# rockcarry/ffcnn

Measured on AMD Instinct MI355X. Metric: frames/sec yolo-fastest-1.1 @320x320 batch-64 per GPU (u8 BGR frames -> net_input's conversion in the first kernel -> full forward: conv stack + YOLO decode + NMS, boxes on rank 0), higher is better.
Workload: dtype f32

## Files before the change

### ffcnn_amd/capi.py

```python
import ctypes as C
import os
import subprocess

import numpy as np

HERE = os.path.dirname(os.path.abspath(__file__))
ROOT = os.path.dirname(HERE)
DATA = os.path.join(ROOT, "data")
CFG = os.path.join(DATA, "yolo-fastest-1.1.cfg")
WEIGHTS = os.path.join(DATA, "yolo-fastest-1.1.weights")

f32p = C.POINTER(C.c_float)


class FFGPU:
    MAX_DET = 128
    MERGE_LDS_SLOTS = 1024
    KEEP_ALL, COMPAT_V6, NO_GRAPH, NO_FUSE, HOST_DETS, SPLIT2, CONCURRENT, BF16_PW = 1, 2, 4, 8, 16, 32, 64, 128
    FEAT_FLAT, FEAT_MEAN, FEAT_MAX = 0, 1, 2
    POST_NONE, POST_SOFTMAX, POST_L2 = 0, 1, 2
    TOPK_MAX = 16
    RELABEL_KEEP_SCORE, RELABEL_LABEL_SCORE = 0, 1
    RELABEL_ENTRIES, RELABEL_MERGED = 0, 1
    K_AUTO, K_GENERIC, K_DW_STREAM, K_DW_LDS, K_PW_MFMA, K_PW_GEMM, _K6, K_DENSE_SMALL, K_IGEMM, K_PW_BF16, K_GROUP_THIN, K_PW_X3, K_CONV_X3, K_PW_X3T = range(14)
# ... 196 lines not shown
PREVIEW_KEEP_BARS = 1
PREVIEW_MAX_SIDE, PREVIEW_MAX_PANES = 8192, 4096
MOTION_DETS, MOTION_ROW, MOTION_WORDS, MOTION_MAX_SIDE = 128, 16, 8, 8192
MOTION_GATE_INVERT = 1
MOTION_ENTRIES, MOTION_MERGED = 0, 1
MOTION_ROW_HEADER = ("frame", "changed", "active", "x0", "y0", "x1", "y1", "warm")
MOTION_WORDS_HEADER = ("considered", "dropped", "outside", "moving", "warm", "frames")
MOTION_STATE_HEADER = 16
HEAT_MAX, HEAT_DETS, HEAT_ROW = 2 ** 31 - 1, 128, 8
HEAT_ANCHOR, HEAT_BOX = 0, 1
HEAT_NEAREST, HEAT_SMOOTH = 0, 1
HEAT_RAMP_ALPHA = 1
HEAT_ENTRIES, HEAT_MERGED = 0, 1
HEAT_ROW_HEADER = ("considered", "dropped", "outside", "frame", "peak", "saturated")
HEAT_STATE_HEADER = 16
TRAIL_POINTS, TRAILS_DETS, TRAILS_ROW = 32, 128, 16
TRAILS_COAST, TRAILS_TAPER = 1, 2
TRAILS_ENTRIES, TRAILS_MERGED = 0, 1
TRAILS_ROW_HEADER = ("considered", "known", "fresh", "refused", "duplicate", "anonymous", "dropped", "freed", "live", "frame", "appended", "drawn", "clipped")
TRAILS_STATE_HEADER = 16
SEG_ITEMS, SEG_LIMIT, OUTLINE_FIXED = 512, 1 << 20, 80
OUTLINE_ZONES, OUTLINE_LINES, OUTLINE_TICKS, OUTLINE_MARKERS, OUTLINE_ALARM = 1, 2, 4, 8, 16
TEXT_MAX, TEXT_ITEMS, TEXT_OPAQUE = 44, 256, 1
CAPTION_DETS = 128
CAPTION_NAME, CAPTION_SCORE, CAPTION_ID, CAPTION_OPAQUE = 1, 2, 4, 8
CAPTION_ENTRIES, CAPTION_MERGED = 0, 1
SCENE_ZONES, SCENE_LINES, ZONE_VERTS, ZONES_DETS, ZONES_ROW = 8, 8, 8, 128, 64
ZONES_NONE, ZONES_TYPE, ZONES_IDS = 0, 1, 2
ZONES_GATE_INVERT = 1
ZONES_ENTRIES, ZONES_MERGED = 0, 1
ZONES_EVENTS_HEADER = ("considered", "known", "fresh", "refused", "duplicate", "anonymous", "dropped", "freed", "live", "frame")
ZONES_STATE_HEADER = 144
TRACK_DETS = 128
TRACK_ENTRIES, TRACK_MERGED = 0, 1
TRACK_IDS_HEADER = ("considered", "matched", "born", "refused", "dropped", "freed", "live", "frame")
CROP_F32, CROP_U8 = 0, 1
CROP_ENTRIES, CROP_MERGED = 0, 1
REDACT_FILL, REDACT_MOSAIC = 0, 1
REDACT_OUTSIDE = 1
REDACT_ENTRIES, REDACT_MERGED = 0, 1
BLUR_OUTSIDE = 1
BLUR_ENTRIES, BLUR_MERGED = 0, 1
DRAW_ENTRIES, DRAW_MERGED = 0, 1
YUV_BT601_LIMITED, YUV_BT601_FULL, YUV_BT709_LIMITED, YUV_BT709_FULL = 0, 1, 2, 3

assert C.sizeof(LAYER) == 120 and C.sizeof(NET) == 104 and C.sizeof(BBOX) == 24
assert C.sizeof(FrameDets) == 16 + 24 * FFGPU.MAX_DET
assert C.sizeof(BgrFrame) == 24 and C.sizeof(Nv12Frame) == 40 and C.sizeof(Tile) == 16 and C.sizeof(TileRect) == 16
assert C.sizeof(DrawStyle) == 24 and C.sizeof(CropSpec) == 72 and C.sizeof(Crop) == 48
assert C.sizeof(TrackSpec) == 32 and C.sizeof(Track) == 48
assert C.sizeof(FeatureSpec) == 16 and C.sizeof(Label) == 8 and C.sizeof(RelabelSpec) == 16
assert C.sizeof(Gallery) == 40 and C.sizeof(RedactSpec) == 40 and C.sizeof(BlurSpec) == 40
assert C.sizeof(TextItem) == 64 and C.sizeof(CaptionSpec) == 48
assert C.sizeof(SegItem) == 32 and C.sizeof(OutlineSpec) == 40
assert C.sizeof(TrailPoint) == 12 and C.sizeof(TrailSlot) == 416 and C.sizeof(TrailsSpec) == 64
assert C.sizeof(HeatSpec) == 56 and C.sizeof(HeatBlendSpec) == 48
assert C.sizeof(MotionSpec) == 64
assert C.sizeof(Zone) == 96 and C.sizeof(Line) == 32 and C.sizeof(Scene) == 1040 and C.sizeof(ZonesSpec) == 32 and C.sizeof(ZoneSlot) == 64

BOX_DTYPE = np.dtype([("type", "<i4"), ("score", "<f4"), ("x1", "<f4"), ("y1", "<f4"), ("x2", "<f4"), ("y2", "<f4")])
DETS_DTYPE = np.dtype([("count", "<i4"), ("ncand", "<i4"), ("overflow", "<i4"), ("nfull", "<i4"),
                       ("box", BOX_DTYPE, (FFGPU.MAX_DET,))])
CROP_DTYPE = np.dtype([("target", "<i4"), ("box", "<i4"), ("type", "<i4"), ("score", "<f4"), ("x0", "<i4"), ("y0", "<i4"), ("w", "<i4"), ("h", "<i4"),
                       ("sw", "<i4"), ("sh", "<i4"), ("s1", "<i4"), ("s2", "<i4")])
TRACK_DTYPE = np.dtype([("id", "<i4"), ("type", "<i4"), ("score", "<f4"), ("x1", "<f4"), ("y1", "<f4"), ("x2", "<f4"), ("y2", "<f4"),
                        ("hits", "<i4"), ("missed", "<i4"), ("born", "<i4"), ("det", "<i4"), ("reserved", "<i4")])
ZONE_SLOT_DTYPE = np.dtype([("id", "<i4"), ("px", "<f4"), ("py", "<f4"), ("inside", "<i4"), ("last", "<i4"), ("reserved", "<i4", (3,)), ("since", "<i4", (8,))])
TRAIL_POINT_DTYPE = np.dtype([("x", "<i4"), ("y", "<i4"), ("frame", "<i4")])
TRAIL_SLOT_DTYPE = np.dtype([("id", "<i4"), ("last", "<i4"), ("n", "<i4"), ("head", "<i4"), ("cx", "<i4"), ("cy", "<i4"), ("reserved", "<i4", (2,)),
                             ("ring", TRAIL_POINT_DTYPE, (32,))])
LABEL_DTYPE = np.dtype([("index", "<i4"), ("value", "<f4")])
TEXT_ITEM_DTYPE = np.dtype([("x", "<i4"), ("y", "<i4"), ("fg", "u1", (4,)), ("bg", "u1", (4,)), ("scale", "u1"), ("flags", "u1"), ("len", "u1"), ("reserved", "u1"),
                            ("text", "u1", (44,))])
SEG_ITEM_DTYPE = np.dtype([("x0", "<i4"), ("y0", "<i4"), ("x1", "<i4"), ("y1", "<i4"), ("color", "u1", (4,)), ("thickness", "u1"), ("dash", "u1"), ("flags", "u1"),
                           ("reserved", "u1"), ("reserved2", "<i4", (2,))])

EXPORTS = ["net_load", "net_free", "net_input", "net_forward", "net_dump", "net_profile", "groupconv",
           "ffgpu_device_count", "ffgpu_set_device", "ffgpu_last_error", "ffgpu_build_info",
           "ffgpu_net_weights_dev", "ffgpu_net_weights_commit",
           "ffgpu_exec_create", "ffgpu_exec_destroy", "ffgpu_exec_batch", "ffgpu_exec_arena_bytes",
           "ffgpu_exec_kernel_count", "ffgpu_exec_work_model", "ffgpu_exec_set_scale", "ffgpu_exec_forward_dev", "ffgpu_exec_forward_host",
           "ffgpu_exec_forward_bgr_dev", "ffgpu_exec_forward_bgr_frames_dev", "ffgpu_exec_forward_nv12_frames_dev", "ffgpu_exec_dets_dev", "ffgpu_exec_dets_host", "ffgpu_exec_set_ring", "ffgpu_exec_set_ring_strided", "ffgpu_exec_read_dets", "ffgpu_exec_read_layer", "ffgpu_exec_hash_layers",
           "ffgpu_exec_read_boxes", "ffgpu_exec_cand_capacity", "ffgpu_exec_graph_captures",
           "ffgpu_exec_profile", "ffgpu_exec_profile_steps", "ffgpu_exec_step_model", "ffgpu_groupconv_dev", "ffgpu_groupconv_kernel_name", "ffgpu_groupconv_time_dev", "ffgpu_irb_dev", "ffgpu_irb_flags_dev", "ffgpu_irb_plan_text", "ffgpu_irb_thin_launch_text", "ffgpu_irb_stage_plan_text", "ffgpu_front_plan_text", "ffgpu_irb_instantiations", "ffgpu_knobs_text", "ffgpu_dwpw_dev", "ffgpu_packed_records_bytes", "ffgpu_pack_records", "ffgpu_unpack_records",
           "ffgpu_shard_range", "ffgpu_node_create", "ffgpu_node_destroy", "ffgpu_node_ndev", "ffgpu_node_shard", "ffgpu_node_set_scale",
           "ffgpu_node_input_dev", "ffgpu_node_input_slot_dev", "ffgpu_node_depth", "ffgpu_node_rccl_ranks", "ffgpu_node_forward", "ffgpu_node_forward_host",
           "ffgpu_node_submit", "ffgpu_node_wait", "ffgpu_node_run",
           "ffgpu_merge_tiles_scratch_bytes", "ffgpu_merge_tiles_dev", "ffgpu_exec_merge_tiles", "ffgpu_exec_merged_dev", "ffgpu_exec_read_merged",
           "ffgpu_exec_read_merged_boxes", "ffgpu_tile_plan",
           "ffgpu_draw_boxes_bgr_dev", "ffgpu_draw_boxes_nv12_dev", "ffgpu_exec_draw_bgr", "ffgpu_exec_draw_nv12",
           "ffgpu_crop_table_bytes", "ffgpu_crop_slot_bytes", "ffgpu_crop_boxes_bgr_dev", "ffgpu_crop_boxes_nv12_dev", "ffgpu_exec_crop_bgr", "ffgpu_exec_crop_nv12",
           "ffgpu_crops_to_source_dev",
           "ffgpu_track_state_bytes", "ffgpu_track_reset_dev", "ffgpu_track_boxes_dev", "ffgpu_exec_track",
           "ffgpu_feature_dim", "ffgpu_exec_feature_dim", "ffgpu_features_dev", "ffgpu_exec_features", "ffgpu_topk_dev", "ffgpu_crops_relabel_dev",
           "ffgpu_exec_relabel",
           "ffgpu_match_workspace_bytes", "ffgpu_match_dev", "ffgpu_gallery_enroll_dev",
           "ffgpu_redact_boxes_bgr_dev", "ffgpu_redact_boxes_nv12_dev", "ffgpu_exec_redact_bgr", "ffgpu_exec_redact_nv12",
           "ffgpu_blur_boxes_bgr_dev", "ffgpu_blur_boxes_nv12_dev", "ffgpu_exec_blur_bgr", "ffgpu_exec_blur_nv12",
           "ffgpu_zones_state_bytes", "ffgpu_scene_check", "ffgpu_zones_reset_dev", "ffgpu_zones_boxes_dev", "ffgpu_exec_zones",
           "ffgpu_font_builtin", "ffgpu_draw_text_bgr_dev", "ffgpu_draw_text_nv12_dev", "ffgpu_caption_boxes_dev", "ffgpu_exec_caption_bgr", "ffgpu_exec_caption_nv12",
           "ffgpu_caption_scene_dev",
           "ffgpu_draw_segments_bgr_dev", "ffgpu_draw_segments_nv12_dev", "ffgpu_outline_spec_check", "ffgpu_outline_scene_dev",
           "ffgpu_trails_state_bytes", "ffgpu_trails_spec_check", "ffgpu_trails_reset_dev", "ffgpu_trails_boxes_dev", "ffgpu_exec_trails",
           "ffgpu_heat_state_bytes", "ffgpu_heat_spec_check", "ffgpu_heat_blend_spec_check", "ffgpu_heat_palette", "ffgpu_heat_reset_dev", "ffgpu_heat_boxes_dev",
           "ffgpu_exec_heat", "ffgpu_heat_blend_bgr_dev", "ffgpu_heat_blend_nv12_dev",
           "ffgpu_motion_state_bytes", "ffgpu_motion_spec_check", "ffgpu_motion_reset_dev", "ffgpu_motion_update_bgr_dev", "ffgpu_motion_update_nv12_dev",
           "ffgpu_motion_gate_dev", "ffgpu_exec_motion_gate",
           "ffgpu_preview_spec_check", "ffgpu_preview_rect", "ffgpu_preview_grid", "ffgpu_preview_tile", "ffgpu_preview_bgr_dev", "ffgpu_preview_nv12_dev",
           "ffgpu_warp_spec_check", "ffgpu_warp_mesh_size", "ffgpu_warp_mesh_orient", "ffgpu_warp_mesh_homography", "ffgpu_warp_mesh_lens", "ffgpu_warp_point",
           "ffgpu_warp_tile", "ffgpu_warp_bgr_dev", "ffgpu_warp_nv12_dev"]
DIAG_EXPORTS = ["ffgpu_membench", "ffgpu_pipe_probe", "ffgpu_pipe_probe2", "ffgpu_pipe_probe3", "ffgpu_mfma_floor", "ffgpu_diag_x3_term", "ffgpu_diag_xl_op", "ffgpu_clock_probe"]


def library_path():
    return os.environ.get("FFCNN_HIP_LIB") or os.path.join(HERE, "lib", "libffcnn_hip.so")


def build_library(force=False):
    cmd = ["make", "-C", os.path.join(HERE, "csrc")]
    if force:
        subprocess.check_call(cmd + ["clean"], stdout=subprocess.DEVNULL)
    subprocess.check_call(cmd, stdout=subprocess.DEVNULL)
    return library_path()


_lib = None


def lib():
    global _lib
    if _lib is not None:
        return _lib
    path = library_path()
    if not os.path.exists(path):
        raise RuntimeError("%s is missing: run `python -c 'import __graft_entry__ as g; g.build()'` "
                           "(the HIP extension is the only compute path)" % path)
    L = C.CDLL(path)
    vp, i, sz = C.c_void_p, C.c_int, C.c_size_t
    L.net_load.restype = C.POINTER(NET)
    L.net_load.argtypes = [C.c_char_p, C.c_char_p, i, i]
    L.net_free.argtypes = [C.POINTER(NET)]
    L.net_input.argtypes = [C.POINTER(NET), vp, i, i, f32p, f32p]
    L.net_forward.argtypes = [C.POINTER(NET)]
    L.net_dump.argtypes = [C.POINTER(NET)]
    L.net_profile.argtypes = [C.POINTER(NET)]
    L.groupconv.argtypes = [f32p, f32p, f32p] + [i] * 12 + [C.POINTER(f32p), C.POINTER(i)]
    L.ffgpu_last_error.restype = C.c_char_p
    L.ffgpu_build_info.restype = C.c_char_p
    if b" DIAG " in L.ffgpu_build_info() and os.environ.get("FFCNN_HIP_ALLOW_DIAG") != "1":
        raise RuntimeError("%s is a DIAG (lab) build of libffcnn_hip; set FFCNN_HIP_ALLOW_DIAG=1 to load it on purpose" % path)
    L.ffgpu_set_device.argtypes = [i]
    L.ffgpu_net_weights_dev.argtypes = [C.POINTER(NET), C.POINTER(vp), C.POINTER(sz)]
    L.ffgpu_net_weights_commit.argtypes = [C.POINTER(NET), vp]
    L.ffgpu_exec_create.restype = vp
    L.ffgpu_exec_create.argtypes = [C.POINTER(NET), i, i]
    L.ffgpu_exec_destroy.argtypes = [vp]
    L.ffgpu_exec_batch.argtypes = [vp]
    L.ffgpu_exec_arena_bytes.restype = sz
    L.ffgpu_exec_arena_bytes.argtypes = [vp]
    L.ffgpu_exec_kernel_count.argtypes = [vp]
    L.ffgpu_exec_work_model.argtypes = [vp, C.POINTER(C.c_double), C.POINTER(C.c_double)]
    L.ffgpu_exec_set_scale.argtypes = [vp, i, i]
    L.ffgpu_exec_forward_dev.argtypes = [vp, vp, vp]
    L.ffgpu_exec_forward_host.argtypes = [vp, f32p]
    L.ffgpu_exec_forward_bgr_dev.argtypes = [vp, vp, i, i, f32p, f32p, vp]
    L.ffgpu_exec_forward_bgr_frames_dev.argtypes = [vp, C.POINTER(BgrFrame), i, f32p, f32p, vp]
    L.ffgpu_exec_forward_nv12_frames_dev.argtypes = [vp, C.POINTER(Nv12Frame), i, f32p, f32p, vp]
    L.ffgpu_exec_dets_dev.argtypes = [vp, C.POINTER(vp), C.POINTER(sz)]
    L.ffgpu_exec_dets_host.restype = vp; L.ffgpu_exec_dets_host.argtypes = [vp]
    L.ffgpu_exec_set_ring.argtypes = [vp, vp, C.c_int]
    L.ffgpu_exec_set_ring_strided.argtypes = [vp, vp, C.c_int, C.c_int]
    L.ffgpu_exec_read_dets.argtypes = [vp, vp, i]
    L.ffgpu_exec_read_layer.argtypes = [vp, i, i, f32p, sz]
    L.ffgpu_exec_hash_layers.argtypes = [vp, vp, i]
    L.ffgpu_exec_profile.argtypes = [vp, vp, f32p]
    L.ffgpu_exec_profile_steps.argtypes = [vp, vp, C.POINTER(i), f32p, i]
    L.ffgpu_exec_step_model.argtypes = [vp, C.POINTER(i), C.POINTER(C.c_double), i]
    L.ffgpu_groupconv_dev.argtypes = [vp, vp, vp] + [i] * 15 + [vp]
    L.ffgpu_groupconv_kernel_name.restype = C.c_char_p
    L.ffgpu_groupconv_kernel_name.argtypes = [i] * 10
    L.ffgpu_groupconv_time_dev.restype = C.c_float
    L.ffgpu_groupconv_time_dev.argtypes = [vp, vp, vp] + [i] * 17 + [vp]
    L.ffgpu_irb_dev.restype = C.c_float
    L.ffgpu_irb_dev.argtypes = [vp] * 6 + [i] * 13 + [vp]
    L.ffgpu_irb_flags_dev.restype = C.c_float
    L.ffgpu_irb_flags_dev.argtypes = [vp] * 6 + [i] * 14 + [vp]
    L.ffgpu_irb_thin_launch_text.argtypes = [i] * 12 + [C.c_char_p, i]
    L.ffgpu_irb_plan_text.argtypes = [i] * 12 + [C.c_char_p, i]
    L.ffgpu_irb_stage_plan_text.argtypes = [i] * 7 + [C.c_char_p, i]
    L.ffgpu_front_plan_text.argtypes = [i] * 4 + [C.c_char_p, i]
    L.ffgpu_irb_instantiations.argtypes = [C.c_char_p, i]
    L.ffgpu_knobs_text.argtypes = [C.c_char_p, i]
    L.ffgpu_exec_read_boxes.argtypes = [vp, i, vp, i]
    L.ffgpu_exec_cand_capacity.argtypes = [vp]
    L.ffgpu_exec_graph_captures.argtypes = [vp]
    L.ffgpu_dwpw_dev.restype = C.c_float
    L.ffgpu_dwpw_dev.argtypes = [vp] * 4 + [i] * 10 + [vp]
    L.ffgpu_packed_records_bytes.restype = C.c_size_t
    L.ffgpu_packed_records_bytes.argtypes = [i, i]
    L.ffgpu_pack_records.restype = i
    L.ffgpu_pack_records.argtypes = [vp, i, C.c_long, i, i, vp, vp]
    L.ffgpu_shard_range.argtypes = [i, i, i, C.POINTER(i), C.POINTER(i)]
    L.ffgpu_shard_range.restype = None
    L.ffgpu_node_create.restype = vp
    L.ffgpu_node_create.argtypes = [C.POINTER(NET), i, C.POINTER(i), i, i, i]
    L.ffgpu_node_destroy.argtypes = [vp]
    L.ffgpu_node_ndev.argtypes = [vp]
    L.ffgpu_node_shard.argtypes = [vp, i, C.POINTER(i), C.POINTER(i), C.POINTER(i)]
    L.ffgpu_node_set_scale.argtypes = [vp, i, i]
    L.ffgpu_node_input_dev.restype = vp
    L.ffgpu_node_input_dev.argtypes = [vp, i]
    L.ffgpu_node_input_slot_dev.restype = vp
    L.ffgpu_node_input_slot_dev.argtypes = [vp, i, i]
    L.ffgpu_node_depth.argtypes = [vp]
    if hasattr(L, "ffgpu_node_rccl_ranks"):
        L.ffgpu_node_rccl_ranks.argtypes = [vp]
    L.ffgpu_node_submit.restype = C.c_long
    L.ffgpu_node_submit.argtypes = [vp, f32p]
    L.ffgpu_node_wait.argtypes = [vp, C.c_long, vp]
    L.ffgpu_node_run.argtypes = [vp, C.c_long, vp]
    L.ffgpu_unpack_records.argtypes = [vp, i, i, vp]
    L.ffgpu_node_forward.argtypes = [vp, vp]
    L.ffgpu_node_forward_host.argtypes = [vp, f32p, vp]
    L.ffgpu_merge_tiles_scratch_bytes.restype = sz
    L.ffgpu_merge_tiles_scratch_bytes.argtypes = [i, i]
    L.ffgpu_merge_tiles_dev.argtypes = [vp, vp, i, C.POINTER(Tile), i, i, C.c_float, i, vp, vp, vp, sz, vp]
    L.ffgpu_exec_merge_tiles.argtypes = [vp, C.POINTER(Tile), i, i, vp]
    L.ffgpu_exec_merged_dev.argtypes = [vp, C.POINTER(vp), C.POINTER(sz)]
    L.ffgpu_exec_read_merged.argtypes = [vp, vp, i]
    L.ffgpu_exec_read_merged_boxes.argtypes = [vp, i, vp, i]
    L.ffgpu_tile_plan.argtypes = [i] * 7 + [C.POINTER(TileRect), i]
    L.ffgpu_draw_boxes_bgr_dev.argtypes = [vp, vp, i, C.POINTER(i), C.POINTER(BgrFrame), i, C.POINTER(DrawStyle), vp]
    L.ffgpu_draw_boxes_nv12_dev.argtypes = [vp, vp, i, C.POINTER(i), C.POINTER(Nv12Frame), i, C.POINTER(DrawStyle), vp]
    L.ffgpu_exec_draw_bgr.argtypes = [vp, i, C.POINTER(BgrFrame), i, C.POINTER(DrawStyle), vp]
    L.ffgpu_exec_draw_nv12.argtypes = [vp, i, C.POINTER(Nv12Frame), i, C.POINTER(DrawStyle), vp]
    L.ffgpu_redact_boxes_bgr_dev.argtypes = [vp, vp, i, C.POINTER(i), C.POINTER(BgrFrame), i, C.POINTER(RedactSpec), vp]
    L.ffgpu_redact_boxes_nv12_dev.argtypes = [vp, vp, i, C.POINTER(i), C.POINTER(Nv12Frame), i, C.POINTER(RedactSpec), vp]
    L.ffgpu_exec_redact_bgr.argtypes = [vp, i, C.POINTER(BgrFrame), i, C.POINTER(RedactSpec), vp]
    L.ffgpu_exec_redact_nv12.argtypes = [vp, i, C.POINTER(Nv12Frame), i, C.POINTER(RedactSpec), vp]
    L.ffgpu_blur_boxes_bgr_dev.argtypes = [vp, vp, i, C.POINTER(i), C.POINTER(BgrFrame), C.POINTER(BgrFrame), i, C.POINTER(BlurSpec), vp]
    L.ffgpu_blur_boxes_nv12_dev.argtypes = [vp, vp, i, C.POINTER(i), C.POINTER(Nv12Frame), C.POINTER(Nv12Frame), i, C.POINTER(BlurSpec), vp]
    L.ffgpu_exec_blur_bgr.argtypes = [vp, i, C.POINTER(BgrFrame), C.POINTER(BgrFrame), i, C.POINTER(BlurSpec), vp]
    L.ffgpu_exec_blur_nv12.argtypes = [vp, i, C.POINTER(Nv12Frame), C.POINTER(Nv12Frame), i, C.POINTER(BlurSpec), vp]
    L.ffgpu_crop_table_bytes.restype = sz
    L.ffgpu_crop_table_bytes.argtypes = [i]
    L.ffgpu_crop_slot_bytes.restype = sz
    L.ffgpu_crop_slot_bytes.argtypes = [i, i, i]
    L.ffgpu_crop_boxes_bgr_dev.argtypes = [vp, vp, i, C.POINTER(i), C.POINTER(BgrFrame), i, C.POINTER(CropSpec), vp, vp, i, vp]
    L.ffgpu_crop_boxes_nv12_dev.argtypes = [vp, vp, i, C.POINTER(i), C.POINTER(Nv12Frame), i, C.POINTER(CropSpec), vp, vp, i, vp]
    L.ffgpu_exec_crop_bgr.argtypes = [vp, i, C.POINTER(BgrFrame), i, C.POINTER(CropSpec), vp, vp, i, vp]
    L.ffgpu_exec_crop_nv12.argtypes = [vp, i, C.POINTER(Nv12Frame), i, C.POINTER(CropSpec), vp, vp, i, vp]
    L.ffgpu_crops_to_source_dev.argtypes = [vp, i, vp, vp, i, vp, vp, vp]
    L.ffgpu_track_state_bytes.restype = sz
    L.ffgpu_track_state_bytes.argtypes = [i, i]
    L.ffgpu_track_reset_dev.argtypes = [vp, i, i, i, vp]
    L.ffgpu_track_boxes_dev.argtypes = [vp, vp, i, C.POINTER(i), C.POINTER(i), i, C.POINTER(TrackSpec), vp, i, vp, vp, vp, vp]
    L.ffgpu_exec_track.argtypes = [vp, i, C.POINTER(i), i, C.POINTER(TrackSpec), vp, i, vp, vp, vp, vp]
    L.ffgpu_zones_state_bytes.restype = sz
    L.ffgpu_zones_state_bytes.argtypes = [i, i]
    L.ffgpu_scene_check.argtypes = [C.POINTER(Scene), i]
    L.ffgpu_zones_reset_dev.argtypes = [vp, i, i, i, vp]
    L.ffgpu_zones_boxes_dev.argtypes = [vp, vp, i, C.POINTER(i), C.POINTER(i), i, C.POINTER(ZonesSpec), vp, vp, i, vp, vp, vp, vp, vp]
    L.ffgpu_exec_zones.argtypes = [vp, i, C.POINTER(i), i, C.POINTER(ZonesSpec), vp, vp, i, vp, vp, vp, vp, vp]
    L.ffgpu_font_builtin.restype = None
    L.ffgpu_font_builtin.argtypes = [vp]
    L.ffgpu_draw_text_bgr_dev.argtypes = [vp, i, vp, C.POINTER(BgrFrame), i, vp]
    L.ffgpu_draw_text_nv12_dev.argtypes = [vp, i, vp, C.POINTER(Nv12Frame), i, vp]
    L.ffgpu_caption_boxes_dev.argtypes = [vp, vp, i, C.POINTER(i), i, C.POINTER(CaptionSpec), vp, vp, i, vp]
    L.ffgpu_exec_caption_bgr.argtypes = [vp, i, C.POINTER(BgrFrame), i, C.POINTER(CaptionSpec), vp, vp, i, vp, vp]
    L.ffgpu_exec_caption_nv12.argtypes = [vp, i, C.POINTER(Nv12Frame), i, C.POINTER(CaptionSpec), vp, vp, i, vp, vp]
# ... 1172 lines not shown
                                     act, flags, variant, stream), "ffgpu_groupconv_dev")


def groupconv_time_dev(d_in, d_filt, d_out, batch, iw, ih, ic, groups, pad, stride, fs, fn, act=0, flags=0, variant=0,
                       warmup=5, iters=20, stream=None):
    ow, oh = (iw + 2 * pad - fs) // stride + 1, (ih + 2 * pad - fs) // stride + 1
    us = lib().ffgpu_groupconv_time_dev(d_in, d_filt, d_out, batch, iw, ih, ic, groups, pad, stride, fs, fn, ow, oh, fn,
                                        act, flags, variant, warmup, iters, stream)
    if us < 0:
        raise RuntimeError("ffgpu_groupconv_time_dev failed: %s" % last_error())
    return us


def packed_records_bytes(batch, cap):
    return int(lib().ffgpu_packed_records_bytes(batch, cap))


def pack_records_dev(d_records, nslots, slot_stride_records, batch, cap, d_out, stream=None):
    _check(lib().ffgpu_pack_records(d_records, nslots, slot_stride_records, batch, cap, d_out, stream), "ffgpu_pack_records")


def kernel_name(batch, iw, ih, ic, groups, pad, stride, fs, fn, variant=0):
    return lib().ffgpu_groupconv_kernel_name(batch, iw, ih, ic, groups, pad, stride, fs, fn, variant).decode()


def irb_plan_text(shape, flags=0):
    buf = C.create_string_buffer(1024)
    if lib().ffgpu_irb_plan_text(*shape, flags, buf, len(buf)) < 0:
        raise RuntimeError("ffgpu_irb_plan_text failed: %s" % last_error())
    return buf.value.decode()


def irb_stage_plan_text(batch, iw, ih, blocks, act1=2, actd=2, flags=0):
    buf = C.create_string_buffer(1024)
    if lib().ffgpu_irb_stage_plan_text(batch, iw, ih, blocks, act1, actd, flags, buf, len(buf)) < 0:
        raise RuntimeError("ffgpu_irb_stage_plan_text failed: %s" % last_error())
    return buf.value.decode()


FRONT_FORMS = {"f32": 0, "u8": 1, "bgr_frames": 2, "nv12_frames": 3}


def front_plan_text(batch, pw, ph, form="f32"):
    buf = C.create_string_buffer(256)
    if lib().ffgpu_front_plan_text(batch, pw, ph, FRONT_FORMS[form], buf, len(buf)) < 0:
        raise RuntimeError("ffgpu_front_plan_text failed: %s" % last_error())
    return buf.value.decode()


def irb_instantiations():
    buf = C.create_string_buffer(4096)
    n = lib().ffgpu_irb_instantiations(buf, len(buf))
    if n < 0 or n >= len(buf):
        raise RuntimeError("ffgpu_irb_instantiations failed: %s" % (last_error() if n < 0 else "%d bytes" % n))
    return buf.value.decode().split()


def knobs():
    buf = C.create_string_buffer(1 << 16)
    n = lib().ffgpu_knobs_text(buf, len(buf))
    if n < 0 or n >= len(buf):
        raise RuntimeError("ffgpu_knobs_text failed: %s" % (last_error() if n < 0 else "%d bytes" % n))
    rows = []
    for line in buf.value.decode().splitlines():
        name, kind, dflt, cls, value, text = line.split(" ", 5)
        rows.append({"name": name, "kind": kind, "default": None if dflt == "-" else dflt if dflt == "computed" else int(dflt), "cls": cls, "value": value, "text": text})
    return rows


def dwpw_dev(d_in, d_wd, d_wp, d_out, batch, iw, ih, c, oc, fs, actd=2, actp=0, warmup=0, iters=0, stream=None):
    us = lib().ffgpu_dwpw_dev(d_in, d_wd, d_wp, d_out, batch, iw, ih, c, oc, fs, actd, actp, warmup, iters, stream)
    if us < 0:
        raise RuntimeError("ffgpu_dwpw_dev failed: %s" % last_error())
    return us


def irb_thin_launch_text(shape, flags=0):
    buf = C.create_string_buffer(256)
    if lib().ffgpu_irb_thin_launch_text(*shape, flags, buf, len(buf)) < 0:
        raise RuntimeError("ffgpu_irb_thin_launch_text failed: %s" % last_error())
    return buf.value.decode()


def irb_dev(d_in, d_w1, d_wd, d_w2, d_res, d_out, batch, iw, ih, ic, ec, oc, stride, act1=2, actd=2, act2=0, res_act=0,
            warmup=0, iters=0, stream=None, flags=0):
    us = lib().ffgpu_irb_flags_dev(d_in, d_w1, d_wd, d_w2, d_res, d_out, batch, iw, ih, ic, ec, oc, stride, act1, actd, act2, res_act, flags,
                                   warmup, iters, stream)
    if us < 0:
        raise RuntimeError("ffgpu_irb_dev failed: %s" % last_error())
    return us


def preview_pane(src=None, dst=None):
    p = PreviewPane()
    if src is not None:
        p.sx, p.sy, p.sw, p.sh = (int(v) for v in src)
    if dst is not None:
        p.dx, p.dy, p.dw, p.dh = (int(v) for v in dst)
    return p


def preview_spec(fit=PREVIEW_STRETCH, fill=(0, 0, 0), keep_bars=False):
    sp = PreviewSpec()
    sp.fit, sp.flags = fit, PREVIEW_KEEP_BARS if keep_bars else 0
    sp.fill[:] = (int(fill[0]), int(fill[1]), int(fill[2]), 0)
    return sp


def preview_spec_check(spec):
    _check(lib().ffgpu_preview_spec_check(spec), "ffgpu_preview_spec_check")


def preview_rect(src_w, src_h, dst_w, dst_h, pane, spec, nv12=False):
    out = (C.c_int * 8)()
    _check(lib().ffgpu_preview_rect(src_w, src_h, dst_w, dst_h, pane, spec, int(bool(nv12)), out), "ffgpu_preview_rect")
    return tuple(out)


def preview_grid(npanes, cols, dst_w, dst_h, gap=0, nv12=False):
    arr = (PreviewPane * max(1, npanes))()
    _check(lib().ffgpu_preview_grid(npanes, cols, dst_w, dst_h, gap, int(bool(nv12)), arr), "ffgpu_preview_grid")
    return [PreviewPane.from_buffer_copy(arr[k]) for k in range(npanes)]


def preview_tile():
    out = (C.c_int * 3)()
    _check(lib().ffgpu_preview_tile(out), "ffgpu_preview_tile")
    return tuple(out)


def _preview_panes(panes):
    arr = (PreviewPane * max(1, len(panes)))()
    for k, p in enumerate(panes):
        arr[k] = p
    return arr


def preview_bgr_dev(srcs, dsts, panes, spec, stream=None):
    if not len(srcs) == len(dsts) == len(panes):
        raise ValueError("%d sources, %d destinations and %d panes" % (len(srcs), len(dsts), len(panes)))
    _check(lib().ffgpu_preview_bgr_dev(bgr_frame_table(srcs), bgr_frame_table(dsts), _preview_panes(panes), len(panes), spec, stream), "ffgpu_preview_bgr_dev")


def preview_nv12_dev(srcs, dsts, panes, spec, stream=None):
    if not len(srcs) == len(dsts) == len(panes):
        raise ValueError("%d sources, %d destinations and %d panes" % (len(srcs), len(dsts), len(panes)))
    _check(lib().ffgpu_preview_nv12_dev(nv12_frame_table(srcs), nv12_frame_table(dsts), _preview_panes(panes), len(panes), spec, stream), "ffgpu_preview_nv12_dev")


def warp_spec(filter=WARP_BILINEAR, border=WARP_FILL, fill=(0, 0, 0)):
    sp = WarpSpec()
    sp.filter, sp.border = filter, border
    sp.fill[:] = (int(fill[0]), int(fill[1]), int(fill[2]), 0)
    return sp


def warp_spec_check(spec):
    _check(lib().ffgpu_warp_spec_check(spec), "ffgpu_warp_spec_check")


def warp_mesh_size(dst_w, dst_h, cell):
    out = (C.c_int * 2)()
    _check(lib().ffgpu_warp_mesh_size(dst_w, dst_h, cell, out), "ffgpu_warp_mesh_size")
    return tuple(out)


# ... 71 lines not shown
```

### ffcnn_amd/csrc/ffgpu_conv_kernels.inc

```
#include "ffgpu_dw_stream.inc"
#include "ffgpu_pw_mfma.inc"
#include "ffgpu_pw_gemm32.inc"
#include "ffgpu_pw_bf16.inc"
#include "ffgpu_conv_igemm.inc"
#include "ffgpu_dwpw.inc"
#include "ffgpu_conv_dense.inc"
#include "ffgpu_irb.inc"
#include "ffgpu_irb_thin.inc"
#include "ffgpu_front.inc"
#include "ffgpu_irb_wave.inc"
#include "ffgpu_irb_wave2.inc"
#include "ffgpu_irb_stage.inc"
#include "ffgpu_pw_x3.inc"
#include "ffgpu_pw_x3t.inc"
#include "ffgpu_conv_x3.inc"
#include "ffgpu_dw_lds.inc"
#include "ffgpu_dw_pair.inc"
#include "ffgpu_conv_thin.inc"

struct BareScratch {
    float *p = nullptr; size_t n = 0; int dev = -1;
    float *get(size_t need)
    {
        int d = 0;
// ... 975 lines not shown
}

static ThinP thin_params(const IrbDesc &d)
{
    ThinP p;
    p.in = d.in; p.out = d.out; p.residual = d.residual; p.w1 = d.w1; p.wd = d.wd; p.w2 = d.w2;
    p.W = d.W; p.H = d.H; p.N = d.N;
    p.band = d.plan.band; p.nbands = (d.H + p.band - 1) / p.band;
    p.act1 = act_slope(d.act1); p.actd = act_slope(d.actd); p.act2 = act_slope(d.act2); p.res_act = act_slope(d.res_act);
    p.ntasks = (long)d.N * p.nbands;
    return p;
}

template <int IC, int EC, int OC>
static int irb_thin_launch(const ThinP &p, const IrbPlan &c, hipStream_t s)
{
    hipLaunchKernelGGL((k_irb_thin<IC, EC, OC>), dim3((unsigned)c.grid), dim3(c.block), 0, s, p);
    LAUNCH_OK("irb_thin");
    return 0;
}

static constexpr bool thin_pair_built(int ic, int ncp) { return !(ic == 8 && ncp == 5); }
static int thin_pair_ncp(int W, int ic)
{
    for (int nc = 3; nc <= 5; nc++)
        if (W % nc == 0 && W / nc <= 32) return thin_pair_built(ic, nc) ? nc : 0;
    return 0;
}

struct ThinForm { int ncp, band, nbands; long ntasks; int grid; };
static ThinForm thin_form(const IrbDesc &d)
{
    ThinForm f;
    const int ncp = thin_pair_ncp(d.W, d.ic);
    const bool pair = ncp && d.N >= 2 && (d.flags & FFGPU_CONCURRENT) && knob(K_THIN_PAIR) != 0;
    const int units = pair ? (d.N + 1) / 2 : d.N;
    f.ncp = pair ? ncp : 0;
    f.band = pair ? knob_or(K_THIN_BAND, thin_band(units, d.H)) : d.plan.band;
    f.nbands = (d.H + f.band - 1) / f.band;
    f.ntasks = (long)units * f.nbands;
    f.grid = pair ? (int)((f.ntasks + 3) / 4) : d.plan.grid;
    return f;
}

template <int IC, int EC, int OC>
static int irb_thin_pair_launch(const ThinP &p, const ThinForm &f, hipStream_t s)
{
    if (f.ncp == 3) hipLaunchKernelGGL((k_irb_thin_pair<IC, EC, OC, 3>), dim3((unsigned)f.grid), dim3(256), 0, s, p);
    else if (f.ncp == 4) hipLaunchKernelGGL((k_irb_thin_pair<IC, EC, OC, 4>), dim3((unsigned)f.grid), dim3(256), 0, s, p);
    else if constexpr (thin_pair_built(IC, 5)) hipLaunchKernelGGL((k_irb_thin_pair<IC, EC, OC, 5>), dim3((unsigned)f.grid), dim3(256), 0, s, p);
    else { ffgpu_set_error("irb_thin_pair: no instantiation for %d columns per lane of %d channels", f.ncp, IC); return -1; }
    LAUNCH_OK("irb_thin_pair");
    return 0;
}

typedef int (*IrbThinLaunch)(const ThinP &, const IrbPlan &, hipStream_t);
typedef int (*IrbThinPairLaunch)(const ThinP &, const ThinForm &, hipStream_t);
struct IrbThinKernel { int IC, OC; IrbThinLaunch launch; IrbThinPairLaunch pair; };
static const IrbThinKernel irb_thin_kernels[] = { { 8, 4, irb_thin_launch<8, 8, 4>, irb_thin_pair_launch<8, 8, 4> }, { 4, 4, irb_thin_launch<4, 8, 4>, irb_thin_pair_launch<4, 8, 4> },
                                                  { 8, 8, irb_thin_launch<8, 8, 8>, irb_thin_pair_launch<8, 8, 8> }, { 4, 8, irb_thin_launch<4, 8, 8>, irb_thin_pair_launch<4, 8, 8> } };

static int launch_irb_thin(const IrbDesc &d, hipStream_t s)
{
    ThinP p = thin_params(d);
    const ThinForm f = thin_form(d);
    if (f.ncp) { p.band = f.band; p.nbands = f.nbands; p.ntasks = f.ntasks; }
    for (const IrbThinKernel &k : irb_thin_kernels)
        if (k.IC == d.ic && k.OC == d.oc) return f.ncp ? k.pair(p, f, s) : k.launch(p, d.plan, s);
    ffgpu_set_error("irb_thin: no instantiation for %d -> 8 -> %d channels", d.ic, d.oc);
    return -1;
}

int ffgpu_irb_thin_launch_line(const IrbDesc &d, char *buf, size_t cap)
{
    if (d.plan.family != IRB_THIN) return snprintf(buf, cap, "unsupported");
    const ThinForm f = thin_form(d);
    char key[48];
    if (f.ncp) snprintf(key, sizeof key, "thin_pair<%d,8,%d,%d>", d.ic, d.oc, f.ncp);
    else snprintf(key, sizeof key, "thin<%d,8,%d>", d.ic, d.oc);
    return snprintf(buf, cap, "%s W=%d H=%d N=%d band=%d nbands=%d ntasks=%ld grid=%d block=256", key, d.W, d.H, d.N, f.band, f.nbands, f.ntasks, f.grid);
}

typedef int (*IrbwLaunch)(const IrbwP &, const IrbPlan &, hipStream_t);
struct IrbwKernel { int KS1, OT, S, NSI, NSO; bool big, x3, xl; Knob gate; IrbwLaunch launch; };
#define IRBW_K(ks1, ot, st, nsi, gate) \
    { ks1, ot, st, nsi, 1, true, false, false, gate, irb_launch_t<IrbwP, k_irbw<ks1, ot, st, nsi, true>> }, \
    { ks1, ot, st, nsi, 1, false, false, false, gate, irb_launch_t<IrbwP, k_irbw<ks1, ot, st, nsi, false>> }
static const IrbwKernel irbw_kernels[] = {
    { 2, 1, 1, 3, 2, true, true, false, K_NONE, irb_launch_t<IrbwP, k_irbw2<2, 3, true>> }, { 4, 1, 1, 3, 2, true, true, false, K_NONE, irb_launch_t<IrbwP, k_irbw2<4, 3, true>> },
    { 2, 1, 1, 3, 2, true, false, false, K_NONE, irb_launch_t<IrbwP, k_irbw2<2, 3, false>> }, { 4, 1, 1, 3, 2, true, false, false, K_NONE, irb_launch_t<IrbwP, k_irbw2<4, 3, false>> },
    { 12, 3, 1, 2, 1, true, true, true, K_NONE, irb_launch_t<IrbwP, k_irbw<12, 3, 1, 2, true, true, true>> },
    { 4, 2, 2, 4, 1, true, true, false, K_NONE, irb_launch_t<IrbwP, k_irbw<4, 2, 2, 4, true, true>> },
    { 6, 2, 1, 2, 1, true, true, false, K_NONE, irb_launch_t<IrbwP, k_irbw<6, 2, 1, 2, true, true>> },
    IRBW_K(1, 1, 1, 2, K_NONE), IRBW_K(2, 1, 1, 2, K_NONE), IRBW_K(4, 1, 1, 2, K_NONE), IRBW_K(2, 2, 1, 2, K_NONE), IRBW_K(4, 2, 1, 2, K_NONE),
    IRBW_K(6, 2, 1, 2, K_NONE), IRBW_K(12, 3, 1, 2, K_NONE), IRBW_K(1, 1, 2, 3, K_NONE), IRBW_K(2, 1, 2, 3, K_NONE), IRBW_K(4, 2, 2, 4, K_NONE),
    IRBW_K(6, 3, 2, 3, K_IRBW_S2_633),
    IRBW_K(1, 1, 2, 4, K_IRBW_S2_NSI4), IRBW_K(2, 1, 2, 4, K_IRBW_S2_NSI4),
};
#undef IRBW_K
static const int irbw_nkernels = (int)(sizeof irbw_kernels / sizeof irbw_kernels[0]);

static bool irbw_has_kernel(int KS1, int OT, int S, int NSI)
{
    for (const IrbwKernel &k : irbw_kernels)
        if (k.KS1 == KS1 && k.OT == OT && k.S == S && k.NSI == NSI && k.NSO == 1 && !k.x3) return k.gate == K_NONE || knob(k.gate) != 0;
    return false;
}

static long irbw_ntiles(const IrbDesc &d, int TWq, int TH) { return (long)d.N * ((d.OW + 4 * TWq - 1) / (4 * TWq)) * ((d.OH + TH - 1) / TH); }

static bool irbw_pick(const IrbDesc &d, IrbPlan &c)
{
    if (knob(K_NO_IRBW)) return false;
    if (d.stride != 1 && d.stride != 2) return false;
    if (d.act1 == 3 || d.actd == 3 || d.act2 == 3 || d.res_act == 3) return false;
    if ((size_t)d.ic * d.N * d.H * d.W >= (1u << 30) || (size_t)d.oc * d.N * d.OH * d.OW >= (1u << 30)) return false;
    const int S = d.stride;
    c.KS1 = ((d.ic + 3) & ~3) / 4; c.OT = (d.oc + 15) / 16; c.ngroups = (d.ec + 15) / 16;
    double best = 1e30;
    for (int TWq = 1; TWq <= 8; TWq++) {
        if (TWq > 1 && (TWq - 1) * 4 >= d.OW) break;
        for (int TH = 1; TWq * TH <= 16 && TH <= d.OH + 1; TH++) {
            const int EW = S == 1 ? 4 * TWq + 4 : 8 * TWq + 4, EH = S * (TH - 1) + 3;
            int NSI = (EW * EH + 63) / 64;
            if (NSI < 2) NSI = 2;
            if (S == 2 && NSI < 3) NSI = 3;
            if (NSI > 4 || !irbw_has_kernel(c.KS1, c.OT, S, NSI)) continue;
            const long tiles = irbw_ntiles(d, TWq, TH) / d.N;
            const double cost = (double)tiles * (NSI * (c.KS1 * 128.0 + 500.0) + 4 * (220.0 + c.OT * 128.0)) * (1.0 + 12.0 / EW);
            if (cost < best) { best = cost; c.TWq = TWq; c.TH = TH; c.EW = EW; c.EH = EH; c.NSI = NSI; }
        }
    }
    if (best > 1e29) return false;
    const int ft = knob(K_IRBW_TWQ), fh = knob(K_IRBW_TH);
    if (ft > 0 && fh > 0 && ft * fh <= 16) {
        const int EW = S == 1 ? 4 * ft + 4 : 8 * ft + 4, EH = S * (fh - 1) + 3;
        if (EW * EH <= c.NSI * 64) { c.TWq = ft; c.TH = fh; c.EW = EW; c.EH = EH; }
    }
    const long ntiles = irbw_ntiles(d, c.TWq, c.TH);
    const int regs = c.NSI * c.KS1 * 4 + c.OT * 16 + 2 * (c.KS1 + 4 * c.OT) + 76;
    c.big = regs > 124;
    if (const int f = knob(K_IRBW_BIG); f >= 0) c.big = f != 0;
    if (const int f = S == 2 && c.KS1 == 1 ? knob(K_IRBW_BIG_S2K1) : -1; f >= 0) c.big = f != 0;
    const bool conc = (d.flags & FFGPU_CONCURRENT) != 0;
    const int x3_mask = knob(K_IRBW_X3);
    const int gmax = std::min(8, c.ngroups);
    int G = 1;
    for (int g = 1; g <= gmax; g++) {
        const size_t slot = (size_t)c.OT * 1024, ereg = (size_t)g * 16 * c.NSI * 64;
        if (g > 1 && ereg / slot < (size_t)(g + 1) / 2) continue;
        G = g;
        if (ntiles * g >= knob_or(K_IRBW_GWAVES, conc ? 500 : 1200)) break;
    }
    if (!conc && G > 1 && G < gmax && c.ngroups % G != 0 && (c.ngroups + G) / (G + 1) <= (c.ngroups + G - 1) / G) G++;
    if (d.stride == 1 && c.ngroups == 9 && ntiles >= 400 && ntiles < 512 && gmax >= 4 && !conc && !knob(K_IRBW_NOEXC)) G = 4;
    if (const int f = ntiles >= 256 && ntiles < 1100 ? knob(K_IRBW_G_MID) : 0; f > 0) G = std::min(gmax, f);
    const bool xl_ok = S == 1 && c.KS1 == 12 && c.OT == 3 && c.NSI == 2 && c.big && ((x3_mask >> 3) & 1) != 0;
    if (xl_ok && conc && ntiles < 256) G = std::min(gmax, knob(K_IRBW_G_XL));
    if (const int f = ntiles < 256 ? knob(K_IRBW_G_SMALL) : 0; f > 0) G = std::min(gmax, f);
    const int fg = knob(K_IRBW_G);
    if (fg >= 1 && fg <= gmax) G = fg;
    c.G = G;
    c.NSO = 1;
    c.x3 = S == 1 && c.KS1 == 6 && c.OT == 2 && c.NSI == 2 && c.big && ((x3_mask >> 2) & 1) != 0;
    if (S == 2 && c.KS1 == 4 && c.OT == 2 && c.NSI == 4 && c.big && ((x3_mask >> 4) & 1) != 0) c.x3 = true;
    c.xl = xl_ok && G > 1;
    if (c.xl) c.x3 = true;
    if (G == 1 && S == 1 && c.OT == 1 && (c.KS1 == 2 || c.KS1 == 4) && knob(K_IRBW_NSO) == 2) {
        double best2 = 1e30; int tw2 = 0, th2 = 0;
        for (int TWq = 1; TWq <= 8; TWq++) {
            if (TWq > 1 && (TWq - 1) * 4 >= d.OW) break;
            for (int TH = 1; TWq * TH <= 32 && TH <= d.OH + 1; TH++) {
                if (TWq * TH <= 16 || TWq * ((TH + 1) / 2) > 16) continue;
                const int EW = 4 * TWq + 4, EH = TH + 2;
                if (EW * EH > 192) continue;
                const long tiles = irbw_ntiles(d, TWq, TH) / d.N;
                const double cost = (double)tiles * (3 * (c.KS1 * 128.0 + 500.0) + 2 * 4 * (220.0 + 128.0)) * (1.0 + 12.0 / EW);
                if (cost < best2) { best2 = cost; tw2 = TWq; th2 = TH; }
            }
        }
        const int f2t = knob(K_IRBW2_TWQ), f2h = knob(K_IRBW2_TH);
        if (f2t > 0 && f2h > 0 && f2t * ((f2h + 1) / 2) <= 16 && (4 * f2t + 4) * (f2h + 2) <= 192) { tw2 = f2t; th2 = f2h; best2 = 0; }
        const long nt2 = tw2 ? irbw_ntiles(d, tw2, th2) : 0;
// ... 331 lines not shown
}

size_t ffgpu_irb_pack_floats(const IrbDesc &d) { return irb_planned(d, "irb_pack_floats") ? (size_t)d.plan.pack_floats : 0; }

int ffgpu_irb_pack(const IrbDesc &d, float *pk, hipStream_t s)
{
    const IrbPlan &c = d.plan;
    if (!irb_planned(d, "irb_pack")) return -1;
    if (c.family == IRB_THIN) return 0;
    if (c.family == IRB_WAVE) {
        IrbwPackP q; q.w1 = d.w1; q.wd = d.wd; q.w2 = d.w2; q.pk = pk; q.ic = d.ic; q.ec = d.ec; q.oc = d.oc;
        q.k4 = (d.ic + 3) & ~3; q.OT = c.OT; q.ngroups = c.ngroups; q.x3 = c.x3; q.half = c.half;
        hipLaunchKernelGGL(k_irbw_pack, dim3((c.pack_floats + 255) / 256), dim3(256), 0, s, q);
        LAUNCH_OK("irbw_pack");
        return 0;
    }
    IrbPackP q;
    q.w1 = d.w1; q.wd = d.wd; q.w2 = d.w2; q.pk = pk;
    q.ic = d.ic; q.ec = d.ec; q.oc = d.oc;
    q.k4 = (d.ic + 3) & ~3; q.ECH = c.ECH; q.MT = c.ECH / 16; q.OT = c.OT; q.nchunks = (d.ec + c.ECH - 1) / c.ECH; q.CH = irb_chunk_floats(q.k4, c.ECH, c.OT);
    const int total = q.nchunks * q.CH + q.OT * 32;
    hipLaunchKernelGGL(k_irb_pack, dim3((total + 255) / 256), dim3(256), 0, s, q);
    LAUNCH_OK("irb_pack");
    return 0;
}

static int irb_thin_key(int ic, int oc, char *key, size_t cap) { return snprintf(key, cap, "thin<%d,8,%d>", ic, oc); }
static int irbw_key(const IrbwKernel &k, char *key, size_t cap)
{
    if (k.NSO == 2) return snprintf(key, cap, "irbw2<%d,%d%s>", k.KS1, k.NSI, k.x3 ? ",x3" : "");
    return snprintf(key, cap, "irbw<%d,%d,%d,%d%s%s%s>", k.KS1, k.OT, k.S, k.NSI, k.big ? ",big" : "", k.x3 ? ",x3" : "", k.xl ? ",xl" : "");
}
static int irb_key(const IrbKernel &k, char *key, size_t cap) { return snprintf(key, cap, "irb<%d,%d,%d,%d,%d>", k.MT, k.OT, k.S, k.NW == 8 ? 1 : 2, k.NW); }

int ffgpu_irb_keys(char *buf, size_t cap)
{
    size_t n = 0;
    char key[48];
    auto put = [&]() { n += (size_t)snprintf(n < cap ? buf + n : nullptr, n < cap ? cap - n : 0, "%s\n", key); };
    for (const IrbThinKernel &k : irb_thin_kernels) { irb_thin_key(k.IC, k.OC, key, sizeof key); put(); }
    for (const IrbwKernel &k : irbw_kernels) { irbw_key(k, key, sizeof key); put(); }
    for (const IrbKernel &k : irb_kernels) { irb_key(k, key, sizeof key); put(); }
    return (int)n;
}

int ffgpu_irb_plan_line(const IrbDesc &d, char *buf, size_t cap)
{
    const IrbPlan &c = d.plan;
    char key[48];
    if (c.family == IRB_THIN) {
        const ThinP p = thin_params(d);
        irb_thin_key(d.ic, d.oc, key, sizeof key);
        return snprintf(buf, cap, "%s W=%d H=%d N=%d band=%d nbands=%d act=%g,%g,%g,%g ntasks=%ld lds=%d grid=%d block=%d half=%d pack=%d",
                        key, p.W, p.H, p.N, p.band, p.nbands, p.act1, p.actd, p.act2, p.res_act, p.ntasks, c.lds, c.grid, c.block, c.half, c.pack_floats);
    }
    if (c.family == IRB_WAVE) {
        const IrbwP p = irbw_params(d);
        const IrbwKernel &k = irbw_kernels[c.inst];
        irbw_key(k, key, sizeof key);
        return snprintf(buf, cap, "%s N=%d H=%d W=%d OH=%d OW=%d ic=%d ec=%d oc=%d act=%g,%g,%g,%g tile=%d,%d,%d,%d tiles=%d,%d,%ld ngroups=%d G=%d WPB=%d o_w2=%d o_cs=%d cs_floats=%d "
                        "xl_off=%d red_cap=%d in_elems=%u vec=%d half_last=%d m=%u,%u,%u,%u xcd=%d lds=%d grid=%d block=%d half=%d pack=%d",
                        key, p.N, p.H, p.W, p.OH, p.OW, p.ic, p.ec, p.oc, p.act1, p.actd, p.act2, p.res_act, p.TWq, p.TH, p.EW, p.EH, p.tiles_x, p.tiles_y, p.ntiles, p.ngroups, p.G, p.WPB,
                        p.o_w2, p.o_cs, p.cs_floats, p.xl_off, p.red_cap, p.in_elems, p.vec, p.half_last, p.m_ew, p.m_tx, p.m_ty, p.m_twq, p.xcd, c.lds, c.grid, c.block, c.half, c.pack_floats);
    }
    if (c.family == IRB_WG) {
        const IrbP p = irb_params(d);
        const IrbKernel &k = irb_kernels[c.inst];
        irb_key(k, key, sizeof key);
        return snprintf(buf, cap, "%s N=%d H=%d W=%d OH=%d OW=%d ic=%d ec=%d oc=%d stride=%d act=%g,%g,%g,%g tile=%d,%d,%d,%d,%d,%d NPin=%d NPout=%d tiles=%d,%d,%d "
                        "k4=%d nchunks=%d ECH=%d CH=%d KS=%d red_off=%d vec_store=%d resident=%d inv_nsi=%d lds=%d grid=%d block=%d half=%d pack=%d",
                        key, p.N, p.H, p.W, p.OH, p.OW, p.ic, p.ec, p.oc, p.stride, p.act1, p.actd, p.act2, p.res_act, p.TH, p.TW, p.TWq, p.NF, p.EH, p.EW,
                        p.NPin, p.NPout, p.tiles_x, p.tiles_y, p.ntiles, p.k4, p.nchunks, p.ECH, p.CH, p.KS, p.red_off, p.vec_store, p.resident, p.inv_nsi, c.lds, c.grid, c.block, c.half, c.pack_floats);
    }
    return snprintf(buf, cap, "unsupported");
}

int ffgpu_launch_irb(const IrbDesc &d, hipStream_t s)
{
    const IrbPlan &c = d.plan;
    if (!irb_planned(d, "irb")) return -1;
    if (knob(K_VERBOSE_IRB)) { char line[1024]; ffgpu_irb_plan_line(d, line, sizeof line); fprintf(stderr, "%s\n", line); }
    if (c.family == IRB_THIN) return launch_irb_thin(d, s);
    if (!d.pk) { ffgpu_set_error("irb: constants not packed"); return -1; }
    return c.family == IRB_WAVE ? irbw_kernels[c.inst].launch(irbw_params(d), c, s) : irb_kernels[c.inst].launch(irb_params(d), c, s);
}

static bool irb_stage_params(const IrbDesc *blocks, int B, IrbStageP &p, size_t &lds)
{
    if (B < 2 || B > IRBS_MAXB) return false;
    const IrbDesc &d0 = blocks[0];
    for (int b = 0; b < B; b++) {
        const IrbDesc &d = blocks[b];
        const IrbPlan &c = d.plan;
        if (d.ic != 48 || d.ec != 224 || d.oc != 48 || d.stride != 1 || d.OH != d.H || d.OW != d.W) return false;
        if (d.N != d0.N || d.H != d0.H || d.W != d0.W || d.act1 != d0.act1 || d.actd != d0.actd) return false;
        if (act_slope(d.act2) != 1.f || act_slope(d.res_act) != 1.f) return false;
        if (c.family != IRB_WAVE || !c.xl || !c.x3 || c.half || c.G != IRBS_WAVES || c.KS1 != 12 || c.OT != 3 || c.ngroups != 2 * IRBS_WAVES) return false;
        if (c.region / (c.OT * 1024) < c.G) return false;
    }
    const int plane = d0.H * d0.W, TWq = (d0.W + 3) / 4;
    if (plane > 128 || TWq * d0.H > 32) return false;
    p = IrbStageP{};
    p.B = B; p.N = d0.N; p.H = d0.H; p.W = d0.W;
    p.act1 = act_slope(d0.act1); p.actd = act_slope(d0.actd);
    p.TWq = TWq; p.P = 4 * TWq + 2; p.EP = p.P * (d0.H + 2);
    int total;
    irbw_layout(d0.plan, p.o_w2, p.o_cs, p.cs_floats, total);
    if (p.cs_floats > 2 * IRBS_WAVES * 64 * 4) return false;
    p.e_off = p.cs_floats;
    p.e_slice = std::max(16 * p.EP, 2048);
    p.xi_off = p.e_off + IRBS_WAVES * p.e_slice;
    p.f_off = p.xi_off + 2 * 4 * 64 * IRBW_XL_DW;
    lds = (size_t)(p.f_off + 48 * plane) * sizeof(float);
    p.m_w = umulhi_magic(d0.W); p.m_twq = umulhi_magic(TWq); p.m_plane = umulhi_magic(plane);
    return lds <= IRB_LDS_MAX;
}

bool ffgpu_irb_stage_ok(const IrbDesc *blocks, int B)
{
    IrbStageP p; size_t lds;
    return irb_stage_params(blocks, B, p, lds);
}

int ffgpu_irb_stage_line(const IrbDesc *blocks, int B, bool wanted, char *buf, size_t cap)
{
    IrbStageP p; size_t lds;
    if (!wanted || !irb_stage_params(blocks, B, p, lds)) return snprintf(buf, cap, "blocks B=%d launches=%d", B, B);
    return snprintf(buf, cap, "stage B=%d launches=1 N=%d H=%d W=%d act=%g,%g TWq=%d P=%d EP=%d o_w2=%d o_cs=%d cs_floats=%d e_off=%d e_slice=%d xi_off=%d f_off=%d m=%u,%u,%u lds=%zu grid=%d block=%d",
                    p.B, p.N, p.H, p.W, p.act1, p.actd, p.TWq, p.P, p.EP, p.o_w2, p.o_cs, p.cs_floats, p.e_off, p.e_slice, p.xi_off, p.f_off, p.m_w, p.m_twq, p.m_plane, lds, p.N, IRBS_WAVES * 64);
}

int ffgpu_launch_irb_stage(const IrbDesc *blocks, int B, hipStream_t s)
{
    IrbStageP p; size_t lds;
    if (!irb_stage_params(blocks, B, p, lds)) { ffgpu_set_error("irb_stage: the run of %d blocks does not fit the stage kernel", B); return -1; }
    p.in = blocks[0].in; p.out = blocks[B - 1].out;
    for (int b = 0; b < B; b++) {
        if (!blocks[b].pk) { ffgpu_set_error("irb_stage: constants not packed"); return -1; }
        p.pk[b] = blocks[b].pk;
    }
    if (!p.in || !p.out) { ffgpu_set_error("irb_stage: no tensors"); return -1; }
    if (lds_allow((const void *)k_irb_stage, lds, "irb_stage")) return -1;
    hipLaunchKernelGGL(k_irb_stage, dim3((unsigned)p.N), dim3(IRBS_WAVES * 64), lds, s, p);
    LAUNCH_OK("irb_stage");
    return 0;
}
```

### ffcnn_amd/csrc/ffgpu_dev.hpp

```cpp
#pragma once
#include <hip/hip_runtime.h>
#include <stddef.h>
#include <stdint.h>
#include <vector>
#include "ffgpu_internal.h"
#include "ffgpu_args.hpp"
#include "ffgpu_streams_host.hpp"
#include "ffgpu_track_host.hpp"
#include "ffgpu_zones_host.hpp"
#include "ffgpu_text_host.hpp"
#include "ffgpu_lines_host.hpp"
#include "ffgpu_trails_host.hpp"
#include "ffgpu_heat_host.hpp"
#include "ffgpu_motion_host.hpp"
#include "ffgpu_preview_host.hpp"
#include "ffgpu_warp_host.hpp"

#define FFGPU_CHECK(expr)                                                                   \
    do {                                                                                    \
        hipError_t e_ = (expr);                                                             \
        if (e_ != hipSuccess) {                                                             \
            ffgpu_set_error("%s failed: %s (%s:%d)", #expr, hipGetErrorString(e_), __FILE__, __LINE__); \
            return -1;                                                                      \
        }                                                                                   \
    } while (0)

struct ConvDesc {
    const float *in;
    const float *const *in_ind;
    const float *filt;
    float       *out;
    const float *residual;
    const float *wpack;
    int   N;
    int   iw, ih, ic;
    int   ow, oh, oc;
    int   fs, stride, pad, groups;
    int   act;
    int   res_act;
    int   flags;
    long  in_cs, in_ns, out_cs, out_ns, res_cs, res_ns;
    int   nsplit;
    int   kernel;
    int   x3_mt;
};
#define FFGPU_F_BATCH_INPUT (1 << 30)

static inline int conv_k4(const ConvDesc &d) { return (d.fs * d.fs * (d.ic / d.groups) + 3) & ~3; }

enum { IRB_NONE = 0, IRB_THIN, IRB_WAVE, IRB_WG };
struct IrbPlan {
    int family;
    int inst;
    int half;
    int pack_floats;
    int lds, grid, block;
    int KS1, OT, NSI, NSO, TWq, TH, EW, EH, ngroups, G, WPB, big, x3, xl;
    int xcd, region;
    int TW, NF, ECH, NW, KS, wbufs, red_off;
    int band, front_band;
};
struct IrbDesc {
    const float *in; float *out; const float *residual;
    const float *w1, *wd, *w2;
    int N, H, W, OH, OW, ic, ec, oc, stride;
    int act1, actd, act2, res_act;
    const float *pk;
    int flags;
    IrbPlan plan;
};
bool   ffgpu_irb_plan(IrbDesc &d);
size_t ffgpu_irb_pack_floats(const IrbDesc &d);
int    ffgpu_irb_pack(const IrbDesc &d, float *pk, hipStream_t s);
int    ffgpu_launch_irb(const IrbDesc &d, hipStream_t s);
int    ffgpu_irb_plan_line(const IrbDesc &d, char *buf, size_t cap);
int    ffgpu_irb_thin_launch_line(const IrbDesc &d, char *buf, size_t cap);
int    ffgpu_irb_keys(char *buf, size_t cap);
#define IRBS_MAXB 8
bool   ffgpu_irb_stage_ok(const IrbDesc *blocks, int B);
int    ffgpu_launch_irb_stage(const IrbDesc *blocks, int B, hipStream_t s);
int    ffgpu_irb_stage_line(const IrbDesc *blocks, int B, bool wanted, char *buf, size_t cap);
bool   ffgpu_front_ok(const ConvDesc &c, const IrbDesc &d);
enum InputForm { IN_F32, IN_U8, IN_BGR_FRAMES, IN_NV12_FRAMES, IN_FORMS };
int    ffgpu_launch_front(const ConvDesc &c, const IrbDesc &d, InputForm form, hipStream_t s);
bool   ffgpu_front_nv12_fused();
int    ffgpu_front_plan_line(const IrbDesc &d, InputForm form, char *buf, size_t cap);
int    ffgpu_front_nc(const IrbDesc &d);

bool   ffgpu_dwpw_ok(const ConvDesc &dw, const ConvDesc &pw);
size_t ffgpu_dwpw_pack_floats(const ConvDesc &dw, const ConvDesc &pw);
int    ffgpu_dwpw_pack(const ConvDesc &dw, const ConvDesc &pw, float *pk, hipStream_t s);
int    ffgpu_launch_dwpw(const ConvDesc &dw, const ConvDesc &pw, const float *wpack, hipStream_t s);

size_t ffgpu_pw_pack_floats(const ConvDesc &d);
void   ffgpu_conv_plan(ConvDesc &d);
int    ffgpu_pw_pack(const ConvDesc &d, float *pk, hipStream_t s);

#define FFGPU_YUV_MATRICES { { 16, 298, 409, 100, 208, 516 }, { 0, 256, 359, 88, 183, 454 }, { 16, 298, 459, 55, 136, 541 }, { 0, 256, 403, 48, 120, 475 } }
int  ffgpu_launch_set_frames(FrameDesc *d_tab, const FrameDesc *h_desc, int n, hipStream_t s);
int  ffgpu_launch_input_frames(const FrameDesc *d_tab, bool nv12, float *out, int N, int W, int H, const float mean[3], const float norm[3], hipStream_t s);

struct ExecParams {
    const float *frames;
    int s1, s2;
    ffgpu_frame_dets *ring;
    int ring_slots, ring_stride;
    int bbox_max;
    const unsigned char *bgr;
    long  bgr_frame;
    int   bgr_pitch;
    float mean[3], norm[3];
    const FrameDesc *frames_tab;
};
int  ffgpu_launch_set_params(ExecParams *d_prm, const ExecParams &v, hipStream_t s);
bool ffgpu_conv_supports_ind(const ConvDesc &d);

bool ffgpu_no_device(const char *what);

int         ffgpu_launch_conv(const ConvDesc &d, int variant, hipStream_t s);
const char *ffgpu_conv_kernel_name(const ConvDesc &d, int variant);
int ffgpu_launch_pool(const float *in, float *out, int N, int c, int w, int h, int fs, int stride, int is_max, hipStream_t s);
int ffgpu_launch_spp(const float *in, float *const out[3], const int fs[3], int n, long planes, int w, int h, hipStream_t s);
int ffgpu_launch_upsample(const float *in, float *out, long planes, int w, int h, int stride, hipStream_t s);
int ffgpu_launch_add_act(const float *a, const float *b, float *out, long n, int act, hipStream_t s);
int ffgpu_launch_copy(const float *src, float *dst, long n, hipStream_t s);
int ffgpu_launch_hash64(const float *x, long n, unsigned long long *out, hipStream_t s);
int ffgpu_launch_input_bgr(const unsigned char *bgr, float *out, int N, int w, int h, int W, int H,
                           int sw, int sh, int s1, int s2, const float mean[3], const float norm[3], hipStream_t s);

struct YoloHead {
    const float *in;
    int   w, h, classes;
    int   anchors[3][2];
    float thresh, scale_xy;
    int   key_base;
};
int ffgpu_launch_yolo(const YoloHead &hd, int N, int netw, int neth, BBOX *cand, int *cand_key, int *ncand, int cap, int *ring_ctr, hipStream_t s);
int ffgpu_launch_nms(const BBOX *cand, const int *cand_key, int *ncand, int cap, BBOX *full, void *scratch,
                     ffgpu_frame_dets *dets, ffgpu_frame_dets *dets_host, const int *ring_ctr, int N,
                     float thresh, int use_min, const ExecParams *prm, hipStream_t s);
#define FFGPU_NMS_LDS_CAP 8192
bool ffgpu_nms_in_lds(int cap_pow2);
int ffgpu_launch_clear(int *ncand, int N, int *ring_ctr, hipStream_t s);

int    ffgpu_merge_build_tab(const char *what, const ffgpu_tile *tiles, int ntiles, int nimages, std::vector<int> &tab, std::vector<int> *off);
size_t ffgpu_merge_tab_bytes(int ntiles);
int    ffgpu_launch_set_ints(int *d_dst, const int *h_src, int n, hipStream_t s);
int    ffgpu_launch_merge_tiles(const int *d_tab, const std::vector<int> &tab, const ffgpu_frame_dets *recs, const BBOX *lists, int stride,
                                float thresh, int use_min, ffgpu_frame_dets *out_recs, BBOX *out_lists, void *scratch, hipStream_t s);

int ffgpu_draw_style_check(const char *what, const ffgpu_draw_style *st, unsigned pal[256], int *npal);
int ffgpu_launch_draw(bool nv12, const DetSource &src, const std::vector<DrawTarget> &targets, const unsigned pal[256], int npal, int thickness, hipStream_t s);

struct CropPlan {
    int   out_w, out_h, form, per_target, nclasses, num, den;
    float min_score, mean[3], norm[3];
    unsigned char classes[256];
};
// ... 50 lines not shown
```

### ffcnn_amd/csrc/ffgpu_exec.hip

```cpp
#include <algorithm>
#include <cstdarg>
#include <cstdint>
#include <cstdio>
#include <cstdlib>
#include <cstring>
#include <map>
#include <mutex>
#include <string>
#include <type_traits>
#include <vector>

#include "ffgpu_dev.hpp"
#include "ffgpu_knobs.hpp"
#include "ffgpu_plan.hpp"
#include "conv.h"

static thread_local char g_err[512] = "";

extern "C" void ffgpu_set_error(const char *fmt, ...)
{
    va_list ap;
    va_start(ap, fmt);
    vsnprintf(g_err, sizeof g_err, fmt, ap);
    va_end(ap);
// ... 1744 lines not shown
{
    if (iters < 1 || fn != oc) { ffgpu_set_error("groupconv_time_dev: bad arguments"); return -1.f; }
    hipStream_t s = (hipStream_t)stream;
    ConvDesc d;
    fill_desc(d, d_in, d_filt, d_out, batch, iw, ih, ic, groups, pad, stride, fs, ow, oh, oc, act, flags);
    float *pk = nullptr;
    if (variant == FFGPU_K_AUTO && ffgpu_pw_pack_floats(d) > 0) {
        if (hipMalloc(&pk, ffgpu_pw_pack_floats(d) * sizeof(float)) != hipSuccess || ffgpu_pw_pack(d, pk, s)) { ffgpu_set_error("pack failed"); return -1.f; }
        d.wpack = pk;
    }
    hipEvent_t e0, e1;
    if (hipEventCreate(&e0) != hipSuccess || hipEventCreate(&e1) != hipSuccess) { ffgpu_set_error("hipEventCreate failed"); return -1.f; }
    for (int i = 0; i < warmup; i++) if (ffgpu_launch_conv(d, variant, s)) return -1.f;
    (void)hipEventRecord(e0, s);
    for (int i = 0; i < iters; i++) if (ffgpu_launch_conv(d, variant, s)) return -1.f;
    (void)hipEventRecord(e1, s);
    if (hipEventSynchronize(e1) != hipSuccess) { ffgpu_set_error("hipEventSynchronize: %s", hipGetErrorString(hipGetLastError())); return -1.f; }
    float ms = 0.f;
    (void)hipEventElapsedTime(&ms, e0, e1);
    (void)hipEventDestroy(e0); (void)hipEventDestroy(e1);
    return ms * 1000.f / iters;
}

static void irb_fill(IrbDesc &d, int batch, int iw, int ih, int ic, int ec, int oc, int stride, int act1, int actd, int act2, int res_act)
{
    d.N = batch; d.H = ih; d.W = iw; d.OH = (ih + 2 - 3) / stride + 1; d.OW = (iw + 2 - 3) / stride + 1;
    d.ic = ic; d.ec = ec; d.oc = oc; d.stride = stride;
    d.act1 = act1; d.actd = actd; d.act2 = act2; d.res_act = res_act;
}

extern "C" int ffgpu_irb_plan_text(int batch, int iw, int ih, int ic, int ec, int oc, int stride, int act1, int actd, int act2, int res_act, int flags, char *buf, int cap)
{
    if (!buf || cap < 1 || batch < 1 || iw < 1 || ih < 1 || stride < 1) { ffgpu_set_error("irb_plan_text: bad arguments"); return -1; }
    IrbDesc d{};
    irb_fill(d, batch, iw, ih, ic, ec, oc, stride, act1, actd, act2, res_act);
    d.flags = flags & FFGPU_CONCURRENT;
    (void)ffgpu_irb_plan(d);
    return ffgpu_irb_plan_line(d, buf, (size_t)cap);
}

extern "C" int ffgpu_front_plan_text(int batch, int pw, int ph, int form, char *buf, int cap)
{
    if (!buf || cap < 1 || batch < 1 || pw < 1 || ph < 1 || form < 0 || form >= IN_FORMS) { ffgpu_set_error("front_plan_text: bad arguments"); return -1; }
    IrbDesc d{};
    irb_fill(d, batch, pw, ph, 8, 8, 4, 1, 0, 0, 0, 0);
    if (!ffgpu_irb_plan(d) || d.plan.family != IRB_THIN) return snprintf(buf, (size_t)cap, "unsupported");
    return ffgpu_front_plan_line(d, (InputForm)form, buf, (size_t)cap);
}

extern "C" int ffgpu_irb_stage_plan_text(int batch, int iw, int ih, int blocks, int act1, int actd, int flags, char *buf, int cap)
{
    if (!buf || cap < 1 || batch < 1 || iw < 1 || ih < 1 || blocks < 1 || blocks > 64) { ffgpu_set_error("irb_stage_plan_text: bad arguments"); return -1; }
    std::vector<IrbDesc> run((size_t)blocks, IrbDesc{});
    for (IrbDesc &d : run) {
        irb_fill(d, batch, iw, ih, 48, 224, 48, 1, act1, actd, 0, 0);
        d.flags = flags & FFGPU_CONCURRENT;
        if (!ffgpu_irb_plan(d)) return snprintf(buf, (size_t)cap, "unsupported");
    }
    return ffgpu_irb_stage_line(run.data(), blocks, stage_wanted(batch, flags), buf, (size_t)cap);
}

extern "C" int ffgpu_irb_instantiations(char *buf, int cap)
{
    if (!buf || cap < 1) { ffgpu_set_error("irb_instantiations: bad arguments"); return -1; }
    return ffgpu_irb_keys(buf, (size_t)cap);
}

extern "C" int ffgpu_knobs_text(char *buf, int cap)
{
    if (!buf || cap < 1) { ffgpu_set_error("knobs_text: bad arguments"); return -1; }
    return ffgpu_knobs_lines(buf, (size_t)cap);
}

extern "C" int ffgpu_irb_thin_launch_text(int batch, int iw, int ih, int ic, int ec, int oc, int stride, int act1, int actd, int act2, int res_act, int flags, char *buf, int cap)
{
    if (!buf || cap < 1 || batch < 1 || iw < 1 || ih < 1 || stride < 1) { ffgpu_set_error("irb_thin_launch_text: bad arguments"); return -1; }
    IrbDesc d{};
    irb_fill(d, batch, iw, ih, ic, ec, oc, stride, act1, actd, act2, res_act);
    d.flags = flags & FFGPU_CONCURRENT;
    (void)ffgpu_irb_plan(d);
    return ffgpu_irb_thin_launch_line(d, buf, (size_t)cap);
}

extern "C" float ffgpu_irb_dev(const float *d_in, const float *d_w1, const float *d_wd, const float *d_w2,
                               const float *d_res, float *d_out, int batch, int iw, int ih, int ic, int ec, int oc,
                               int stride, int act1, int actd, int act2, int res_act, int warmup, int iters, void *stream)
{
    return ffgpu_irb_flags_dev(d_in, d_w1, d_wd, d_w2, d_res, d_out, batch, iw, ih, ic, ec, oc, stride, act1, actd, act2, res_act, 0, warmup, iters, stream);
}

extern "C" float ffgpu_irb_flags_dev(const float *d_in, const float *d_w1, const float *d_wd, const float *d_w2,
                                     const float *d_res, float *d_out, int batch, int iw, int ih, int ic, int ec, int oc,
                                     int stride, int act1, int actd, int act2, int res_act, int flags, int warmup, int iters, void *stream)
{
    hipStream_t s = (hipStream_t)stream;
    IrbDesc d{};
    d.in = d_in; d.out = d_out; d.residual = d_res; d.w1 = d_w1; d.wd = d_wd; d.w2 = d_w2;
    irb_fill(d, batch, iw, ih, ic, ec, oc, stride, act1, actd, act2, res_act);
    d.flags = flags & FFGPU_CONCURRENT;
    if (!d_in || !d_out || !d_w1 || !d_wd || !d_w2 || !ffgpu_irb_plan(d)) { ffgpu_set_error("irb_dev: unsupported block shape"); return -1.f; }
    float *pk = nullptr;
    if (hipMalloc(&pk, ffgpu_irb_pack_floats(d) * sizeof(float)) != hipSuccess) { ffgpu_set_error("irb_dev: hipMalloc failed"); return -1.f; }
    d.pk = pk;
    float us = 0.f;
    int rc = ffgpu_irb_pack(d, pk, s);
    if (!rc && iters <= 0) rc = ffgpu_launch_irb(d, s);
    if (!rc && iters > 0) {
        hipEvent_t e0, e1;
        (void)hipEventCreate(&e0); (void)hipEventCreate(&e1);
        for (int i = 0; i < warmup && !rc; i++) rc = ffgpu_launch_irb(d, s);
        (void)hipEventRecord(e0, s);
        for (int i = 0; i < iters && !rc; i++) rc = ffgpu_launch_irb(d, s);
        (void)hipEventRecord(e1, s);
        (void)hipEventSynchronize(e1);
        float ms = 0.f;
        (void)hipEventElapsedTime(&ms, e0, e1);
        us = ms * 1000.f / iters;
        (void)hipEventDestroy(e0); (void)hipEventDestroy(e1);
    }
    (void)hipStreamSynchronize(s);
    (void)hipFree(pk);
    return rc ? -1.f : us;
}

extern "C" float ffgpu_dwpw_dev(const float *d_in, const float *d_wd, const float *d_wp, float *d_out, int batch, int iw, int ih,
                                int c, int oc, int fs, int actd, int actp, int warmup, int iters, void *stream)
{
    hipStream_t s = (hipStream_t)stream;
    ConvDesc dw, pw;
    fill_desc(dw, d_in, d_wd, nullptr, batch, iw, ih, c, c, fs / 2, 1, fs, iw, ih, c, actd, 0);
    fill_desc(pw, nullptr, d_wp, d_out, batch, iw, ih, c, 1, 0, 1, 1, iw, ih, oc, actp, 0);
    if (!d_in || !d_wd || !d_wp || !d_out || !ffgpu_dwpw_ok(dw, pw)) { ffgpu_set_error("dwpw_dev: unsupported layer pair"); return -1.f; }
    float *pk = nullptr;
    if (hipMalloc(&pk, ffgpu_dwpw_pack_floats(dw, pw) * sizeof(float)) != hipSuccess) { ffgpu_set_error("dwpw_dev: hipMalloc failed"); return -1.f; }
    float us = 0.f;
    int rc = ffgpu_dwpw_pack(dw, pw, pk, s);
    if (!rc && iters <= 0) rc = ffgpu_launch_dwpw(dw, pw, pk, s);
    if (!rc && iters > 0) {
        hipEvent_t e0, e1;
        (void)hipEventCreate(&e0); (void)hipEventCreate(&e1);
        for (int i = 0; i < warmup && !rc; i++) rc = ffgpu_launch_dwpw(dw, pw, pk, s);
        (void)hipEventRecord(e0, s);
        for (int i = 0; i < iters && !rc; i++) rc = ffgpu_launch_dwpw(dw, pw, pk, s);
        (void)hipEventRecord(e1, s);
        (void)hipEventSynchronize(e1);
        float ms = 0.f;
        (void)hipEventElapsedTime(&ms, e0, e1);
        us = ms * 1000.f / iters;
        (void)hipEventDestroy(e0); (void)hipEventDestroy(e1);
    }
    (void)hipStreamSynchronize(s);
    (void)hipFree(pk);
    return rc ? -1.f : us;
}

struct HostConvScratch { float *in = nullptr, *filt = nullptr, *out = nullptr; size_t in_n = 0, filt_n = 0, out_n = 0; int dev = -1; };

static int grow(float **p, size_t *have, size_t need)
{
    if (*have >= need) return 0;
    (void)hipFree(*p);
    *p = nullptr; *have = 0;
    FFGPU_CHECK(hipMalloc(p, need * sizeof(float)));
    *have = need;
    return 0;
}
// ... 26 lines not shown
```

### ffcnn_amd/csrc/ffgpu_irb_wave2.inc

```
#ifndef IRBW2_X3_KS2_MINB
#define IRBW2_X3_KS2_MINB 2
#endif
template <int KS1, int NSI, bool X3>
__global__ void __launch_bounds__(256, (X3 && KS1 == 2) ? IRBW2_X3_KS2_MINB : 2) k_irbw2(IrbwP p)
{
    constexpr int NM = X3 ? irbw_x3_nm(KS1) : 1;
    extern __shared__ __attribute__((aligned(16))) float smem[];
    const int tid = threadIdx.x, lane = tid & 63, wid = __builtin_amdgcn_readfirstlane(tid >> 6);
    const int kq = lane >> 4, jq = lane & 15;
    const float fl_act1 = act_floor(p.act1), fl_actd = act_floor(p.actd), fl_act2 = act_floor(p.act2), fl_res = act_floor(p.res_act);
    constexpr int NPw = NSI * 64, NQ = NSI * 16, NSO = 2;
    const int ecp = p.ngroups * 16;
    const float *Wd = smem, *Sb1 = smem + ecp * 12, *Sb2 = Sb1 + ecp * 2;
    float *Ew = smem + p.cs_floats + wid * (16 * NPw);
    const v4f_w z = { 0.f, 0.f, 0.f, 0.f };

    const int cs4 = p.cs_floats >> 2, nthr = (int)blockDim.x;
    v4f_w cst[3];
#pragma unroll
    for (int u = 0; u < 3; u++) cst[u] = irbw_ld<v4f_w>(p.pk, (unsigned)(p.o_cs + 4 * min(tid + u * nthr, cs4 - 1)) * 4u);

    const int tile = (p.xcd ? irbw_xcd_block((int)blockIdx.x, (int)gridDim.x) : (int)blockIdx.x) * p.WPB + wid;
    const bool active = tile < (int)p.ntiles;
    const int tt = active ? tile : 0;
    const int trow = irbw_div(tt, p.m_tx), tx_i = tt - trow * p.tiles_x;
    const int n = irbw_div(trow, p.m_ty), ty_i = trow - n * p.tiles_y;
    const int oy0 = ty_i * p.TH, ox0 = tx_i * p.TWq * 4;
    const int gy0 = oy0 - 1, gx0 = ox0 - 1;
    const bool interior = gy0 >= 0 && gx0 >= 0 && gy0 + p.EH <= p.H && gx0 + p.EW <= p.W;

    v4f_w xin[NSI][KS1];
    unsigned mbits = 0;
    {
        const int plane = p.H * p.W;
        bool anyfix = false;
#pragma unroll
        for (int si = 0; si < NSI; si++) {
            const int e = si * 64 + 4 * jq;
            const int iy = (int)__umulhi((unsigned)e, p.m_ew), ix = e - iy * p.EW;
            const int gy = gy0 + iy, gx = gx0 + ix;
            if (!interior) {
                const bool rowok = (iy < p.EH) & ((unsigned)gy < (unsigned)p.H);
#pragma unroll
                for (int q = 0; q < 4; q++) mbits |= (rowok & ((unsigned)(gx + q) < (unsigned)p.W)) ? 1u << (si * 4 + q) : 0u;
            }
            const int rowidx = (n * p.H + min(max(gy, 0), p.H - 1)) * p.W + gx;
#pragma unroll
            for (int ks = 0; ks < KS1; ks++) {
                const int idx = min(4 * ks + kq, p.ic - 1) * (p.N * plane) + rowidx;
                const int cl = min(max(idx, 0), (int)p.in_elems - 4);
                anyfix |= cl != idx;
                xin[si][ks] = irbw_ld<v4f_w>(p.in, (unsigned)cl * 4u);
            }
        }
        if (anyfix) {
#pragma unroll
            for (int si = 0; si < NSI; si++) {
                const int e = si * 64 + 4 * jq;
                const int iy = (int)__umulhi((unsigned)e, p.m_ew), ix = e - iy * p.EW;
                const int rowidx = (n * p.H + min(max(gy0 + iy, 0), p.H - 1)) * p.W + gx0 + ix;
#pragma unroll
                for (int ks = 0; ks < KS1; ks++) {
                    const int idx = min(4 * ks + kq, p.ic - 1) * (p.N * plane) + rowidx;
                    const int d = min(max(idx, 0), (int)p.in_elems - 4) - idx;
                    if (d != 0) {
                        const v4f_w l = xin[si][ks];
                        v4f_w w = z;
#pragma unroll
                        for (int q = 0; q < 4; q++) {
                            const int s = q - d;
                            w[q] = s == 0 ? l.x : (s == 1 ? l.y : (s == 2 ? l.z : (s == 3 ? l.w : 0.f)));
                        }
                        xin[si][ks] = w;
                    }
                }
            }
        }
    }
    if (4 * (KS1 - 1) + kq >= p.ic) {
#pragma unroll
        for (int si = 0; si < NSI; si++) xin[si][KS1 - 1] = z;
    }
    unsigned xp[X3 ? NSI : 1][4][3][X3 ? KS1 / 2 : 1];
    if (X3) {
        float amax = 0.f;
#pragma unroll
        for (int si = 0; si < NSI; si++)
#pragma unroll
            for (int ks = 0; ks < KS1; ks++) amax = x3_amax3(x3_amax3(amax, xin[si][ks][0], xin[si][ks][1]), xin[si][ks][2], xin[si][ks][3]);
        auto split_tile = [&](auto INF) {
#pragma unroll
            for (int si = 0; si < NSI; si++)
#pragma unroll
                for (int q = 0; q < 4; q++) {
                    unsigned b[3][KS1];
#pragma unroll
                    for (int ks = 0; ks < KS1; ks++) {
                        const float x = xin[si][ks][q];
                        const float r = x3_resid_t<decltype(INF)::value>(x);
                        const float r2 = x3_resid2(r);
                        b[0][ks] = __float_as_uint(x); b[1][ks] = __float_as_uint(r); b[2][ks] = __float_as_uint(r2);
                    }
#pragma unroll
                    for (int pt = 0; pt < 3; pt++)
#pragma unroll
                        for (int pr = 0; pr < KS1 / 2; pr++) xp[si][q][pt][pr] = __builtin_amdgcn_perm(b[pt][2 * pr + 1], b[pt][2 * pr], 0x07060302u);
                }
        };
        if (X3_INF_X_FUSED && x3_wave_has_inf(amax)) split_tile(std::true_type{}); else split_tile(std::false_type{});
    }
    auto bop = [&](int si, int q, int m) -> v8bf_w2 {
        u4_w2 u;
#pragma unroll
        for (int d = 0; d < 4; d++) {
            const IrbwX3Term t = irbw_x3_term(KS1, m, d);
            u[d] = t.wp < 0 ? 0u : xp[X3 ? si : 0][q][t.xp][X3 ? t.pair : 0];
        }
        return __builtin_bit_cast(v8bf_w2, u);
    };
    int ebase[NSO], nvalid[NSO];
    unsigned pbase[NSO];
    const int typ = irbw_div(jq, p.m_twq), tq = jq - typ * p.TWq;
#pragma unroll
    for (int so = 0; so < NSO; so++) {
        const int ty = 2 * typ + so;
        const bool qvalid = ty < p.TH;
        ebase[so] = qvalid ? ty * p.EW + tq * 4 : 0;
        const int oy = oy0 + ty, ox = ox0 + tq * 4;
        const bool valid = active && qvalid && oy < p.OH && ox < p.OW;
        nvalid[so] = valid ? min(4, p.OW - ox) : 0;
        pbase[so] = valid ? (unsigned)((n * p.OH + oy) * p.OW + ox) : 0u;
    }
    const unsigned ocs = (unsigned)(p.N * p.OH * p.OW);

    struct W1T { float f[X3 ? 1 : KS1]; u4_w2 x[X3 ? NM : 1]; };
    auto loadw = [&](int g, W1T &w1, float (&w2)[4]) {
        if (X3) {
#pragma unroll
            for (int m = 0; m < NM; m++) w1.x[m] = irbw_ld<u4_w2>(p.pk, (unsigned)((g * NM + m) * 64 + lane) * 16u);
        } else {
#pragma unroll
            for (int ks = 0; ks < KS1; ks++) w1.f[ks] = irbw_ld<float>(p.pk, (unsigned)((g * KS1 + ks) * 64 + lane) * 4u);
        }
#pragma unroll
        for (int i = 0; i < 4; i++) w2[i] = irbw_ld<float>(p.pk, (unsigned)(p.o_w2 + (g * 4 + i) * 64 + lane) * 4u);
    };
    W1T w1a, w1b;
    float w2a[4], w2b[4];
    loadw(0, w1a, w2a);

#pragma unroll
    for (int u = 0; u < 3; u++) if (tid + u * nthr < cs4) reinterpret_cast<v4f_w *>(smem)[tid + u * nthr] = cst[u];
    for (int i = tid + 3 * nthr; i < cs4; i += nthr)
        reinterpret_cast<v4f_w *>(smem)[i] = irbw_ld<v4f_w>(p.pk, (unsigned)(p.o_cs + 4 * i) * 4u);
    __syncthreads();

    v4f_w acc[NSO][4];
#pragma unroll
    for (int so = 0; so < NSO; so++)
#pragma unroll
        for (int q = 0; q < 4; q++) acc[so][q] = z;
    const unsigned mb = interior ? 0xffffffffu : mbits;

    auto group = [&](int g, const W1T &w1, const float (&w2)[4]) {
        const float *sbp = Sb1 + (g * 4 + kq) * 8;
        const v4f_w S4 = *reinterpret_cast<const v4f_w *>(sbp), B4 = *reinterpret_cast<const v4f_w *>(sbp + 4);
        const v2f_w sc[2] = { { S4.x, S4.y }, { S4.z, S4.w } }, bi[2] = { { B4.x, B4.y }, { B4.z, B4.w } };
#pragma unroll
        for (int si = 0; si < NSI; si++) {
            v4f_w a4[4] = { z, z, z, z };
            if (X3) {
#pragma unroll
                for (int m = 0; m < NM; m++) {
                    const v8bf_w2 A = __builtin_bit_cast(v8bf_w2, w1.x[m]);
#pragma unroll
                    for (int q = 0; q < 4; q++) a4[q] = __builtin_amdgcn_mfma_f32_16x16x32_bf16(A, bop(si, q, m), a4[q], 0, 0, 0);
                }
            } else {
#pragma unroll
                for (int ks = 0; ks < KS1; ks++) {
                    a4[0] = __builtin_amdgcn_mfma_f32_16x16x4f32(w1.f[ks], xin[si][ks].x, a4[0], 0, 0, 0);
                    a4[1] = __builtin_amdgcn_mfma_f32_16x16x4f32(w1.f[ks], xin[si][ks].y, a4[1], 0, 0, 0);
                    a4[2] = __builtin_amdgcn_mfma_f32_16x16x4f32(w1.f[ks], xin[si][ks].z, a4[2], 0, 0, 0);
                    a4[3] = __builtin_amdgcn_mfma_f32_16x16x4f32(w1.f[ks], xin[si][ks].w, a4[3], 0, 0, 0);
                }
            }
#pragma unroll
            for (int rp = 0; rp < 2; rp++) {
                v2f_w y[4];
#pragma unroll
                for (int q = 0; q < 4; q++) {
                    const v2f_w a = rp == 0 ? (v2f_w){ a4[q].x, a4[q].y } : (v2f_w){ a4[q].z, a4[q].w };
                    const v2f_w t = a * sc[rp] + bi[rp];
                    const v2f_w u = t * p.act1;
                    const bool in = (mb >> (si * 4 + q)) & 1u;
                    y[q] = (v2f_w){ in ? act_max(t.x, u.x, fl_act1) : 0.f, in ? act_max(t.y, u.y, fl_act1) : 0.f };
                }
                float *dst = Ew + ((2 * kq + rp) * 2 * NQ + si * 16 + jq) * 4;
                *reinterpret_cast<v4f_w *>(dst) = (v4f_w){ y[0].x, y[0].y, y[1].x, y[1].y };
                *reinterpret_cast<v4f_w *>(dst + NQ * 4) = (v4f_w){ y[2].x, y[2].y, y[3].x, y[3].y };
            }
        }
#pragma unroll
        for (int m = 0; m < 2; m++) {
            const int pr = 2 * kq + m;
            const float *wdp = Wd + (g * 8 + pr) * 24;
            v4f_w T[6];
#pragma unroll
            for (int i = 0; i < 6; i++) T[i] = *reinterpret_cast<const v4f_w *>(wdp + 4 * i);
            const v2f_w tap[9] = { { T[0].x, T[0].y }, { T[0].z, T[0].w }, { T[1].x, T[1].y }, { T[1].z, T[1].w }, { T[2].x, T[2].y },
                                   { T[2].z, T[2].w }, { T[3].x, T[3].y }, { T[3].z, T[3].w }, { T[4].x, T[4].y } };
            const v2f_w sd = { T[4].z, T[4].w }, bd = { T[5].x, T[5].y };
            const float *ep = Ew + (pr * 2 * NQ + (ebase[0] >> 2)) * 4;
            v2f_w dv[NSO][4];
#pragma unroll
            for (int so = 0; so < NSO; so++)
#pragma unroll
                for (int q = 0; q < 4; q++) dv[so][q] = (v2f_w){ 0.f, 0.f };
#pragma unroll
            for (int r = 0; r < 4; r++) {
                const float *row = ep + r * p.EW;
                v2f_w x[6];
#pragma unroll
                for (int i = 0; i < 3; i++) {
                    const v4f_w u = *reinterpret_cast<const v4f_w *>(row + ((i & 1) * NQ + (i >> 1)) * 4);
                    x[2 * i] = (v2f_w){ u.x, u.y }; x[2 * i + 1] = (v2f_w){ u.z, u.w };
                }
                if (r < 3) {
#pragma unroll
                    for (int q = 0; q < 4; q++)
#pragma unroll
                        for (int kx = 0; kx < 3; kx++) dv[0][q] += tap[r * 3 + kx] * x[q + kx];
                }
                if (r >= 1) {
#pragma unroll
                    for (int q = 0; q < 4; q++)
#pragma unroll
                        for (int kx = 0; kx < 3; kx++) dv[1][q] += tap[(r - 1) * 3 + kx] * x[q + kx];
                }
            }
#pragma unroll
            for (int so = 0; so < NSO; so++) {
                v2f_w bq[4];
#pragma unroll
                for (int q = 0; q < 4; q++) {
                    const v2f_w t = dv[so][q] * sd + bd;
                    const v2f_w u = t * p.actd;
                    bq[q] = (v2f_w){ act_max(t.x, u.x, fl_actd), act_max(t.y, u.y, fl_actd) };
                }
#pragma unroll
                for (int j = 0; j < 2; j++) {
                    const float a = w2[2 * m + j];
                    acc[so][0] = __builtin_amdgcn_mfma_f32_16x16x4f32(a, j ? bq[0].y : bq[0].x, acc[so][0], 0, 0, 0);
                    acc[so][1] = __builtin_amdgcn_mfma_f32_16x16x4f32(a, j ? bq[1].y : bq[1].x, acc[so][1], 0, 0, 0);
                    acc[so][2] = __builtin_amdgcn_mfma_f32_16x16x4f32(a, j ? bq[2].y : bq[2].x, acc[so][2], 0, 0, 0);
                    acc[so][3] = __builtin_amdgcn_mfma_f32_16x16x4f32(a, j ? bq[3].y : bq[3].x, acc[so][3], 0, 0, 0);
                }
            }
        }
    };

    if (active) {
        for (int g = 0; g < p.ngroups; g += 2) {
            loadw(min(g + 1, p.ngroups - 1), w1b, w2b);
            __builtin_amdgcn_sched_barrier(0);
            group(g, w1a, w2a);
            if (g + 1 < p.ngroups) {
                loadw(min(g + 2, p.ngroups - 1), w1a, w2a);
                __builtin_amdgcn_sched_barrier(0);
                group(g + 1, w1b, w2b);
            }
        }
    }

    const bool lin_out = p.act2 == 1.f && p.res_act == 1.f;
    auto rows_out = [&](auto MODE) {
        constexpr int M = decltype(MODE)::value;
#pragma unroll
        for (int so = 0; so < NSO; so++) {
            v4f_w res[4];
            if (M == 0 || (M == 2 && p.residual)) {
#pragma unroll
                for (int r = 0; r < 4; r++) {
                    const unsigned off = ((unsigned)min(4 * kq + r, p.oc - 1) * ocs + pbase[so]) * 4u;
                    if (p.vec == 4) res[r] = irbw_ld<v4f_w>(p.residual, nvalid[so] == 4 ? off : 0u);
                    else {
#pragma unroll
                        for (int q = 0; q < 4; q++) res[r][q] = irbw_ld<float>(p.residual, q < nvalid[so] ? off + 4u * q : 0u);
                    }
                }
            }
#pragma unroll
            for (int r = 0; r < 4; r++) {
                const int o = 4 * kq + r, oo = min(o, p.oc - 1);
                const v2f_w sb = *reinterpret_cast<const v2f_w *>(Sb2 + 2 * oo);
                v4f_w v = pw_fma4_apart(acc[so][0][r], acc[so][1][r], acc[so][2][r], acc[so][3][r], sb.x, sb.y);
                if (M == 0) v += res[r];
                if (M == 2) {
#pragma unroll
                    for (int q = 0; q < 4; q++) {
                        v[q] = irbw_act(v[q], p.act2, fl_act2);
                        if (p.residual) v[q] = irbw_act(v[q] + res[r][q], p.res_act, fl_res);
                    }
                }
                const unsigned off = ((unsigned)oo * ocs + pbase[so]) * 4u;
                if (o < p.oc) {
                    if (p.vec == 4) { if (nvalid[so] == 4) irbw_st<v4f_w>(p.out, off, v); }
                    else {
#pragma unroll
                        for (int q = 0; q < 4; q++) if (q < nvalid[so]) irbw_st<float>(p.out, off + 4u * q, v[q]);
                    }
                }
            }
        }
    };
    if (lin_out && p.residual) rows_out(std::integral_constant<int, 0>());
    else if (lin_out) rows_out(std::integral_constant<int, 1>());
    else rows_out(std::integral_constant<int, 2>());
}
```

### ffcnn_amd/csrc/ffgpu_knobs.hpp

```cpp
#pragma once
#include <assert.h>
#include <limits.h>
#include <stdio.h>
#include <stdlib.h>

enum KnobKind { KNOB_INT, KNOB_ON, KNOB_SET, KNOB_TEXT };
enum KnobClass { KNOB_PRODUCT, KNOB_TUNING, KNOB_TEST, KNOB_LAB };
#define KNOB_COMPUTED INT_MIN

#define FFGPU_KNOBS_MAIN(X) \
     \
    X(COMPAT_V6,         "FFCNN_COMPAT_V6",         ON,   0,             PRODUCT, "the reference's v6 behaviour for 5x5 filters (executors and groupconv)") \
    X(NO_GRAPH,          "FFGPU_NO_GRAPH",          ON,   0,             PRODUCT, "eager launches instead of a captured graph (as the flag FFGPU_NO_GRAPH)") \
    X(BF16_PW,           "FFGPU_BF16_PW",           ON,   0,             PRODUCT, "opt-in bf16 inputs for compute-bound pointwise layers; own tolerance (as the flag)") \
    X(NO_FUSE,           "FFGPU_NO_FUSE",           ON,   0,             PRODUCT, "one kernel per layer: no fused blocks, no concat in place, no residual in the conv epilogue (as the flag)") \
    X(BRANCH,            "FFGPU_BRANCH",            ON,   0,             PRODUCT, "first detection head as a parallel graph branch instead of in line") \
    X(DWPW,              "FFGPU_DWPW",              ON,   0,             PRODUCT, "the heads' depthwise + pointwise pairs as one kernel (measured slower)") \
    X(NO_U8_FRONT,       "FFGPU_NO_U8_FRONT",       SET,  0,             PRODUCT, "u8 frames through the staging kernel and the fp32 first kernel even where they could go straight in") \
    X(NV12_FRONT,        "FFGPU_NV12_FRONT",        INT,  KNOB_COMPUTED, PRODUCT, "1: NV12 frames into the NV12 form of k_front where the plan has it, 0: staged; default: the build's measured choice") \
    X(VERBOSE,           "FFGPU_VERBOSE",           SET,  0,             PRODUCT, "print every error to stderr as it is set") \
    X(NODE_PACK_BOXES,   "FFGPU_NODE_PACK_BOXES",   INT,  0,             PRODUCT, "room per frame in a shard's packed record block; 0 or less: 16, the constant of the same name in ffgpu_node.inc") \
    X(NO_IRB,            "FFGPU_NO_IRB",            ON,   0,             TUNING,  "no fused inverted-residual blocks: their three layers as three kernels") \
    X(IRB_MIN_EC,        "FFGPU_IRB_MIN_EC",        INT,  24,            TUNING,  "fewest expanded channels of a block the planner fuses (thin blocks apart)") \
    X(IRB_STAGE,         "FFGPU_IRB_STAGE",         INT,  1,             TUNING,  "runs of 48 -> 224 -> 48 blocks on a small plane as one launch in FFGPU_CONCURRENT executors of 32 frames or more (0: one launch per block)") \
    X(SPLIT_PARTS,       "FFGPU_SPLIT_PARTS",       INT,  2,             TUNING,  "parallel chains of an FFGPU_SPLIT2 executor: 2, 4 or 8 (where the batch divides)") \
    X(NO_INDIRECT,       "FFGPU_NO_INDIRECT",       ON,   0,             TEST,    "the first kernel takes the input address from its arguments, not the parameter block: graphs keyed by input pointer") \
     \
    X(FORCE_GENERIC,     "FFGPU_FORCE_GENERIC",     INT,  0,             PRODUCT, "the reference-order generic kernel for every convolution") \
    X(PW_X3,             "FFGPU_PW_X3",             INT,  1,             PRODUCT, "0: never pick the split-bf16 pointwise kernel k_pw_x3") \
    X(PWX3_MIN_IC,       "FFGPU_PWX3_MIN_IC",       INT,  192,           TUNING,  "k_pw_x3: fewest input channels AUTO takes it for") \
    X(PWX3_MIN_OC,       "FFGPU_PWX3_MIN_OC",       INT,  256,           TUNING,  "k_pw_x3: fewest output channels") \
    X(PWX3_MIN_P,        "FFGPU_PWX3_MIN_P",        INT,  65536,         TUNING,  "k_pw_x3: fewest pixels") \
    X(PWX3_MT,           "FFGPU_PWX3_MT",           INT,  0,             TUNING,  "k_pw_x3: 16-row blocks per wave, 1 / 2 / 4 (0: 4)") \
    X(PW_X3T,            "FFGPU_PW_X3T",            INT,  1,             PRODUCT, "0: never pick the tiled split-bf16 GEMM k_pw_x3t") \
    X(PWX3T_MIN_IC,      "FFGPU_PWX3T_MIN_IC",      INT,  128,           TUNING,  "k_pw_x3t: fewest input channels AUTO takes it for") \
    X(PWX3T_MIN_OC,      "FFGPU_PWX3T_MIN_OC",      INT,  192,           TUNING,  "k_pw_x3t: fewest output channels") \
    X(PWX3T_MIN_P,       "FFGPU_PWX3T_MIN_P",       INT,  65536,         TUNING,  "k_pw_x3t: fewest pixels") \
    X(PWXT_TM,           "FFGPU_PWXT_TM",           INT,  256,           TUNING,  "k_pw_x3t: channels per workgroup tile, 256 or 128 (frozen with a plan: ConvDesc::x3_mt)") \
    X(PWXT_NARROW,       "FFGPU_PWXT_NARROW",       INT,  1,             TUNING,  "k_pw_x3t: 0 switches the narrow tiles of the partial last round off") \
    X(PWXT_PERSIST,      "FFGPU_PWXT_PERSIST",      INT,  0,             TUNING,  "k_pw_x3t: persistent workgroups over the main tiles") \
    X(PWXT_NT,           "FFGPU_PWXT_NT",           INT,  -1,            TUNING,  "k_pw_x3t: non-temporal output stores never (0) / always (1); -1: outputs of 128 MB and more") \
    X(PWXT_DBG,          "FFGPU_PWXT_DBG",          INT,  0,             LAB,     "k_pw_x3t: ablation mask handed to the kernel (wrong results)") \
    X(PW_X3S,            "FFGPU_PW_X3S",            INT,  1,             PRODUCT, "0: never pick the pointwise form of k_conv_x3 (pw_x3s)") \
    X(PWX3S_MIN_IC,      "FFGPU_PWX3S_MIN_IC",      INT,  96,            TUNING,  "pw_x3s: fewest input channels AUTO takes it for") \
    X(PWX3S_MIN_OC,      "FFGPU_PWX3S_MIN_OC",      INT,  64,            TUNING,  "pw_x3s: fewest output channels") \
    X(PWX3S_MIN_WGS,     "FFGPU_PWX3S_MIN_WGS",     INT,  64,            TUNING,  "pw_x3s: fewest workgroups") \
    X(IG_X3,             "FFGPU_IG_X3",             INT,  1,             PRODUCT, "0: never pick the split-bf16 dense 3x3 kernel k_conv_x3") \
    X(IGX3_S2,           "FFGPU_IGX3_S2",           INT,  1,             TUNING,  "k_conv_x3: 0 keeps the stride-2 layers on the fp32 implicit GEMM") \
    X(IGX3_NW,           "FFGPU_IGX3_NW",           INT,  0,             TUNING,  "k_conv_x3: waves per workgroup, 4 or 8 (0: 8 at stride 2, else 4)") \
    X(IGX3_MT,           "FFGPU_IGX3_MT",           INT,  0,             TUNING,  "k_conv_x3: 16-row blocks per wave, 1 / 2 / 4 (0: by shape; frozen with a plan: ConvDesc::x3_mt)") \
    X(IGX3_MT4_WGS,      "FFGPU_IGX3_MT4_WGS",      INT,  192,           TUNING,  "k_conv_x3: fewest workgroups that four blocks per wave must leave") \
    X(IGX3_MIN_IC,       "FFGPU_IGX3_MIN_IC",       INT,  16,            TUNING,  "k_conv_x3: fewest input channels AUTO takes it for") \
    X(IGX3_MIN_WGS,      "FFGPU_IGX3_MIN_WGS",      INT,  160,           TUNING,  "k_conv_x3: fewest workgroups AUTO takes it for") \
    X(PWG_MIN_OC,        "FFGPU_PWG_MIN_OC",        INT,  128,           TUNING,  "k_pw_gemm32: fewest output channels AUTO takes it for") \
    X(PWG_MIN_IC,        "FFGPU_PWG_MIN_IC",        INT,  64,            TUNING,  "k_pw_gemm32: fewest input channels") \
    X(NO_PW_GEMM,        "FFGPU_NO_PW_GEMM",        INT,  0,             PRODUCT, "never pick k_pw_gemm32: k_pw_mfma instead") \
    X(NO_IGEMM,          "FFGPU_NO_IGEMM",          INT,  0,             TUNING,  "never pick the implicit GEMMs (k_conv_igemm, the dense form of k_conv_x3)") \
    X(NO_GROUP_THIN,     "FFGPU_NO_GROUP_THIN",     INT,  0,             TUNING,  "never pick k_conv_thin for grouped layers of few channels per group") \
    X(NO_DW_PAIR,        "FFGPU_NO_DW_PAIR",        INT,  0,             PRODUCT, "depthwise layers on k_dw_lds instead of k_dw_pair") \
    X(NO_CONV_FIRST,     "FFGPU_NO_CONV_FIRST",     INT,  0,             PRODUCT, "the first layer on the dense small-channel kernel instead of k_conv_first") \
    X(CONV_FIRST_MIN_PX, "FFGPU_CONV_FIRST_MIN_PX", INT,  262144,        TUNING,  "k_conv_first: fewest output pixels of the batch") \
    X(NO_POOL2X2,        "FFGPU_NO_POOL2X2",        INT,  0,             TEST,    "2x2 / stride 2 max pooling on the general pool kernel") \
     \
    X(IGEMM_NOVEC,       "FFGPU_IGEMM_NOVEC",       INT,  0,             TUNING,  "k_conv_igemm: no vector form of the gather") \
    X(IGEMM_SPLIT,       "FFGPU_IGEMM_SPLIT",       INT,  0,             TUNING,  "k_conv_igemm: split-K factor 1 .. 16 (0: by tile count; frozen with a plan: ConvDesc::nsplit)") \
    X(DW_U,              "FFGPU_DW_U",              INT,  4,             TUNING,  "k_dw3_stream: rows per step, 1 / 2 / 4") \
    X(DW_BAND,           "FFGPU_DW_BAND",           INT,  4,             TUNING,  "k_dw3_stream: rows per wave task (0: enough tasks to fill the chip)") \
    X(DW_NT,             "FFGPU_DW_NT",             INT,  -1,            PRODUCT, "k_dw3_stream: stream past the caches never (0) / always (1); -1: outputs of 128 MB and more") \
    X(DW_XCD,            "FFGPU_DW_XCD",            INT,  0,             TUNING,  "k_dw3_stream: walk the tasks XCD by XCD") \
    X(DWP_NI,            "FFGPU_DWP_NI",            INT,  0,             TUNING,  "k_dw_pair: frames per workgroup, at most (0: by shape)") \
    X(DWL_BH,            "FFGPU_DWL_BH",            INT,  0,             TUNING,  "k_dw_lds: rows per band (0: by shape)") \
    X(DWL_NPL,           "FFGPU_DWL_NPL",           INT,  0,             TUNING,  "k_dw_lds: planes per item (0: by shape)") \
    X(PWG_WM,            "FFGPU_PWG_WM",            INT,  0,             TUNING,  "k_pw_gemm32: waves per workgroup, 4 or 8 (0: 8 from 248 output channels; part of the packed image)") \
    X(PWG_NARROW,        "FFGPU_PWG_NARROW",        INT,  1,             TUNING,  "k_pw_gemm32: 0 switches the narrow tiles of the partial last round off") \
    X(PWG_DBG,           "FFGPU_PWG_DBG",           INT,  0,             LAB,     "k_pw_gemm32: ablation mask handed to the kernel (wrong results)") \
     \
    X(NO_THIN,           "FFGPU_NO_THIN",           INT,  0,             PRODUCT, "8-channel blocks on the wave kernel instead of k_irb_thin") \
    X(THIN_BAND,         "FFGPU_THIN_BAND",         INT,  KNOB_COMPUTED, TUNING,  "k_irb_thin: rows per wave; default by batch and height (thin_band)") \
    X(THIN_PAIR,         "FFGPU_THIN_PAIR",         INT,  1,             TUNING,  "k_irb_thin: 0 keeps FFGPU_CONCURRENT executors off the paired form (two frames per wave, 3 / 4 / 5 columns per lane); read at launch") \
    X(FRONT_BAND,        "FFGPU_FRONT_BAND",       INT,  KNOB_COMPUTED, TUNING,  "k_front: rows per wave; default as FFGPU_THIN_BAND") \
    X(NO_FRONT,          "FFGPU_NO_FRONT",          INT,  0,             PRODUCT, "layers 0-3 as k_conv_first + k_irb_thin instead of k_front") \
    X(FRONT_MIN_PX,      "FFGPU_FRONT_MIN_PX",      INT,  262144,        TUNING,  "k_front: fewest output pixels of the batch") \
    X(FRONT_NC,          "FFGPU_FRONT_NC",          INT,  3,             PRODUCT, "k_front: output columns per lane, 3 where a row fits a wave that way, or 4") \
    X(NO_IRBW,           "FFGPU_NO_IRBW",           INT,  0,             PRODUCT, "fused blocks on the workgroup kernel k_irb instead of the wave-autonomous k_irbw") \
    X(IRBW_S2_633,       "FFGPU_IRBW_S2_633",       INT,  1,             TUNING,  "k_irbw: 0 hides the stride-2 form for 24 input / 48 output channels from the planner") \
    X(IRBW_S2_NSI4,      "FFGPU_IRBW_S2_NSI4",      INT,  0,             TUNING,  "k_irbw: 1 lets the planner take the four-strip halo for the thin stride-2 blocks") \
    X(IRBW_TWQ,          "FFGPU_IRBW_TWQ",          INT,  0,             TUNING,  "k_irbw: tile width in quads (with FFGPU_IRBW_TH; 0: searched)") \
    X(IRBW_TH,           "FFGPU_IRBW_TH",           INT,  0,             TUNING,  "k_irbw: tile height (with FFGPU_IRBW_TWQ; 0: searched)") \
    X(IRBW_BIG,          "FFGPU_IRBW_BIG",          INT,  -1,            TUNING,  "k_irbw: the 256-register form never (0) / always (1); -1: by register need") \
    X(IRBW_BIG_S2K1,     "FFGPU_IRBW_BIG_S2K1",     INT,  -1,            TUNING,  "k_irbw: as FFGPU_IRBW_BIG for the stride-2 blocks of at most 4 input channels alone") \
    X(IRBW_GWAVES,       "FFGPU_IRBW_GWAVES",       INT,  KNOB_COMPUTED, TUNING,  "k_irbw: waves a launch wants before the group split stops; default 1200, 500 with FFGPU_CONCURRENT") \
    X(IRBW_NOEXC,        "FFGPU_IRBW_NOEXC",        INT,  0,             TUNING,  "k_irbw: without the measured exception (four waves on the 20x20 blocks)") \
    X(IRBW_G_MID,        "FFGPU_IRBW_G_MID",        INT,  0,             TUNING,  "k_irbw: group split for 256 .. 1099 tiles (0: as computed)") \
    X(IRBW_X3,           "FFGPU_IRBW_X3",           INT,  30,            PRODUCT, "fused blocks: expand GEMM as split-bf16 products, one bit per shape: 0: 8 input channels, 1: 16, 2: 24, 3: 48 (split tile in LDS), 4: the 40 -> 20 stride-2 block") \
    X(IRBW_G_XL,         "FFGPU_IRBW_G_XL",         INT,  7,             TUNING,  "k_irbw: group split of the LDS-resident form with several chains in flight") \
    X(IRBW_G_SMALL,      "FFGPU_IRBW_G_SMALL",      INT,  0,             TUNING,  "k_irbw: group split under 256 tiles (0: as computed)") \
    X(IRBW_G,            "FFGPU_IRBW_G",            INT,  0,             TUNING,  "k_irbw: group split, wins over everything (0: as computed)") \
    X(IRBW_NSO,          "FFGPU_IRBW_NSO",          INT,  2,             TUNING,  "k_irbw2: anything but 2 keeps the planner off the two-strip kernel") \
    X(IRBW2_TWQ,         "FFGPU_IRBW2_TWQ",         INT,  0,             TUNING,  "k_irbw2: tile width in quads (with FFGPU_IRBW2_TH; 0: searched)") \
    X(IRBW2_TH,          "FFGPU_IRBW2_TH",          INT,  0,             TUNING,  "k_irbw2: tile height (with FFGPU_IRBW2_TWQ; 0: searched)") \
    X(IRBW2_MIN_TILES,   "FFGPU_IRBW2_MIN_TILES",   INT,  768,           TUNING,  "k_irbw2: fewest tiles the planner takes it for") \
    X(IRBW_WPB,          "FFGPU_IRBW_WPB",          INT,  0,             TUNING,  "k_irbw: tiles per workgroup without a group split, 1 .. 8 (0: 4 or 8 by LDS)") \
    X(IRBW_HALF,         "FFGPU_IRBW_HALF",         INT,  1,             PRODUCT, "0: a last group of at most 8 real expanded channels is computed as a whole group") \
    X(IRBW_XCD,          "FFGPU_IRBW_XCD",          INT,  3,             PRODUCT, "fused blocks walk their tiles XCD by XCD; bit 0: one-wave-per-tile launches, bit 1: group-split launches") \
    X(IRBW_FOLD,         "FFGPU_IRBW_FOLD",         INT,  0,             TUNING,  "k_irbw: never widen the reduction region to all G partial sums (folding rounds)") \
    X(IRB_ECH,           "FFGPU_IRB_ECH",           INT,  0,             TUNING,  "k_irb: expanded channels per chunk, 16 or 32 (0: by shape)") \
    X(IRB_RESIDENT,      "FFGPU_IRB_RESIDENT",      INT,  1,             TUNING,  "k_irb: every chunk's constants in LDS never (0) / where it costs no workgroup (1) / wherever they fit (2)") \
    X(IRB_TW,            "FFGPU_IRB_TW",            INT,  0,             TUNING,  "k_irb: tile width (0: the measured table, then the search)") \
    X(IRB_TH,            "FFGPU_IRB_TH",            INT,  0,             TUNING,  "k_irb: tile height for the search (0: any)") \
    X(IRB_NF,            "FFGPU_IRB_NF",            INT,  0,             TUNING,  "k_irb: frames per tile for the search, 1 / 2 / 4 (0: any)") \
    X(IRB_NOTABLE,       "FFGPU_IRB_NOTABLE",       INT,  0,             TUNING,  "k_irb: skip the measured table of tiles, search") \
    X(IRB_NW,            "FFGPU_IRB_NW",            INT,  8,             TUNING,  "k_irb: waves per workgroup, 8 or 4") \
    X(IRB_NOKS,          "FFGPU_IRB_NOKS",          INT,  0,             TUNING,  "k_irb: idle waves take no slices of the channel loop") \
    X(IRB_SKIP,          "FFGPU_IRB_SKIP",          INT,  0,             LAB,     "k_irb: ablation mask, 1 no input loads, 2 no expand, 4 no depthwise / project, 8 no stores (wrong results)") \
    X(IRB_TRACE,         "FFGPU_IRB_TRACE",         INT,  0,             LAB,     "lab builds with -DIRB_TRACE=1: every fused-block launch is followed by its in-kernel timeline on stderr") \
    X(VERBOSE_IRB,       "FFGPU_VERBOSE_IRB",       INT,  0,             LAB,     "print the plan line of every fused-block launch to stderr")

#ifdef FFGPU_DIAG
#define FFGPU_KNOBS_DIAG(X) \
    X(DBG_SKIP,          "FFGPU_DBG_SKIP",          TEXT, 0,             LAB,     "make DIAG=1: \"lo:hi\" drops the launches of layers lo .. hi (wrong results)") \
    X(DBG_KEEP,          "FFGPU_DBG_KEEP",          TEXT, 0,             LAB,     "make DIAG=1: \"lo:hi\" drops every launch but those of layers lo .. hi (wrong results)")
#else
#define FFGPU_KNOBS_DIAG(X)
#endif
#if defined(XT_TRACE) && XT_TRACE
#define FFGPU_KNOBS_XT(X) \
    X(PWXT_TRACE,        "FFGPU_PWXT_TRACE",        TEXT, 0,             LAB,     "builds with -DXT_TRACE=1: file that one traced k_pw_x3t launch dumps its per-tile timeline to")
#else
#define FFGPU_KNOBS_XT(X)
#endif
#define FFGPU_KNOBS(X) FFGPU_KNOBS_MAIN(X) FFGPU_KNOBS_DIAG(X) FFGPU_KNOBS_XT(X)

struct KnobRow { const char *name; KnobKind kind; int dflt; KnobClass cls; const char *text; };
#define X(id, name, kind, dflt, cls, text) K_##id,
enum Knob { FFGPU_KNOBS(X) K_COUNT, K_NONE = -1 };
#undef X
#define X(id, name, kind, dflt, cls, text) { name, KNOB_##kind, dflt, KNOB_##cls, text },
static constexpr KnobRow ffgpu_knob_rows[K_COUNT] = { FFGPU_KNOBS(X) };
#undef X

static inline int knob_int_(const KnobRow &r, int dflt) { const char *v = getenv(r.name); return v && *v ? atoi(v) : dflt; }
static inline int knob(Knob k)
{
    const KnobRow &r = ffgpu_knob_rows[k];
    assert((r.kind == KNOB_INT && r.dflt != KNOB_COMPUTED) || r.kind == KNOB_ON);
    if (r.kind == KNOB_INT) return knob_int_(r, r.dflt);
    const char *v = getenv(r.name);
    return v && atoi(v) != 0;
}
static inline int knob_or(Knob k, int dflt)
{
    const KnobRow &r = ffgpu_knob_rows[k];
    assert(r.kind == KNOB_INT && r.dflt == KNOB_COMPUTED);
    return knob_int_(r, dflt);
}
static inline bool knob_set(Knob k) { assert(ffgpu_knob_rows[k].kind == KNOB_SET); return getenv(ffgpu_knob_rows[k].name) != nullptr; }
static inline const char *knob_text(Knob k) { assert(ffgpu_knob_rows[k].kind == KNOB_TEXT); return getenv(ffgpu_knob_rows[k].name); }

static inline int ffgpu_knobs_lines(char *buf, size_t cap)
{
    static const char *const kinds[] = { "INT", "ON", "SET", "TEXT" }, *const classes[] = { "product", "tuning", "test", "lab" };
    size_t n = 0;
    if (cap) buf[0] = 0;
    for (int k = 0; k < K_COUNT; k++) {
        const KnobRow &r = ffgpu_knob_rows[k];
        const char *const env = getenv(r.name);
        char dflt[16] = "-", val[16];
        if (r.kind == KNOB_INT && r.dflt == KNOB_COMPUTED) snprintf(dflt, sizeof dflt, "computed");
        else if (r.kind != KNOB_TEXT) snprintf(dflt, sizeof dflt, "%d", r.dflt);
        if (r.kind == KNOB_TEXT) snprintf(val, sizeof val, env ? "set" : "unset");
        else if (r.kind == KNOB_SET) snprintf(val, sizeof val, "%d", (int)knob_set((Knob)k));
        else if (r.kind == KNOB_INT && r.dflt == KNOB_COMPUTED && !(env && *env)) snprintf(val, sizeof val, "default");
        else snprintf(val, sizeof val, "%d", r.kind == KNOB_INT && r.dflt == KNOB_COMPUTED ? knob_or((Knob)k, 0) : knob((Knob)k));
        n += (size_t)snprintf(n < cap ? buf + n : nullptr, n < cap ? cap - n : 0, "%s %s %s %s %s %s\n", r.name, kinds[r.kind], dflt, classes[r.cls], val, r.text);
    }
    return (int)n;
}
```

### include/ffcnn_hip.h

```cpp
#ifndef FFCNN_AMD_FFCNN_HIP_H
#define FFCNN_AMD_FFCNN_HIP_H

#include <stddef.h>
#include "ffcnn.h"

#ifdef __cplusplus
extern "C" {
#endif

#define FFGPU_MAX_DET   128



typedef struct {
    int  count;
    int  ncand;
    int  overflow;
    int  nfull;
    BBOX box[FFGPU_MAX_DET];
} ffgpu_frame_dets;

typedef struct ffgpu_exec ffgpu_exec;

#define FFGPU_KEEP_ALL   1
// ... 57 lines not shown
} ffgpu_nv12_frame;

int ffgpu_exec_forward_nv12_frames_dev(ffgpu_exec *ex, const ffgpu_nv12_frame *frames, int nframes,
                                       const float mean[3], const float norm[3], void *stream);

int ffgpu_exec_dets_dev(ffgpu_exec *ex, void **dev_ptr, size_t *bytes);
const ffgpu_frame_dets *ffgpu_exec_dets_host(ffgpu_exec *ex);
int ffgpu_exec_set_ring(ffgpu_exec *ex, void *dev_ring, int slots);
int ffgpu_exec_set_ring_strided(ffgpu_exec *ex, void *dev_ring, int slots, int slot_records);
int ffgpu_exec_read_dets(ffgpu_exec *ex, ffgpu_frame_dets *host_out, int max_frames);
int ffgpu_exec_read_boxes(ffgpu_exec *ex, int frame, BBOX *host_out, int cap);
int ffgpu_exec_cand_capacity(const ffgpu_exec *ex);
int ffgpu_exec_graph_captures(const ffgpu_exec *ex);

int ffgpu_exec_read_layer(ffgpu_exec *ex, int layer, int frame, float *host_out, size_t cap_floats);

int ffgpu_exec_hash_layers(ffgpu_exec *ex, unsigned long long *host_out, int cap);

int ffgpu_exec_profile(ffgpu_exec *ex, const float *d_frames, float us_by_kind[LAYER_TYPE_TOTOAL]);

int ffgpu_exec_profile_steps(ffgpu_exec *ex, const float *d_frames, int *layer_of, float *us, int cap);
int ffgpu_exec_step_model(const ffgpu_exec *ex, int *layer_of, double *hbm_bytes, int cap);

typedef struct ffgpu_node ffgpu_node;
#define FFGPU_NODE_LOOPBACK 1
#define FFGPU_NODE_DEPTH(n) (((n) & 0xf) << 8)

void        ffgpu_shard_range(int total, int rank, int world, int *lo, int *hi);
ffgpu_node *ffgpu_node_create(NET *net, int ndev, const int *devices, int global_batch, int exec_flags, int node_flags);
void        ffgpu_node_destroy(ffgpu_node *node);
int         ffgpu_node_ndev(const ffgpu_node *node);
int         ffgpu_node_shard(const ffgpu_node *node, int rank, int *lo, int *hi, int *device);
int         ffgpu_node_set_scale(ffgpu_node *node, int s1, int s2);
int         ffgpu_node_depth(const ffgpu_node *node);
int         ffgpu_node_rccl_ranks(const ffgpu_node *node);
float      *ffgpu_node_input_dev(ffgpu_node *node, int rank);
float      *ffgpu_node_input_slot_dev(ffgpu_node *node, int rank, int slot);
int         ffgpu_node_forward(ffgpu_node *node, ffgpu_frame_dets *host_out);
int         ffgpu_node_forward_host(ffgpu_node *node, const float *h_frames, ffgpu_frame_dets *host_out);
long        ffgpu_node_submit(ffgpu_node *node, const float *h_frames);
int         ffgpu_node_wait(ffgpu_node *node, long ticket, ffgpu_frame_dets *host_out);
int         ffgpu_node_run(ffgpu_node *node, long steps, ffgpu_frame_dets *host_out);

int ffgpu_groupconv_dev(const float *d_in, const float *d_filt, float *d_out, int batch,
                        int iw, int ih, int ic, int groups, int pad, int stride,
                        int fs, int fn, int ow, int oh, int oc, int act,
                        int flags, int variant, void *stream);

enum {
    FFGPU_K_AUTO = 0,
    FFGPU_K_GENERIC = 1,
    FFGPU_K_DW_STREAM = 2,
    FFGPU_K_DW_LDS = 3,
    FFGPU_K_PW_MFMA = 4,
    FFGPU_K_PW_GEMM = 5,
    FFGPU_K_DENSE_SMALL = 7,
    FFGPU_K_IGEMM = 8,
    FFGPU_K_PW_BF16 = 9,
    FFGPU_K_GROUP_THIN = 10,
    FFGPU_K_PW_X3 = 11,
    FFGPU_K_CONV_X3 = 12,
    FFGPU_K_PW_X3T = 13
};

const char *ffgpu_groupconv_kernel_name(int batch, int iw, int ih, int ic, int groups, int pad,
                                        int stride, int fs, int fn, int variant);

float ffgpu_groupconv_time_dev(const float *d_in, const float *d_filt, float *d_out, int batch,
                               int iw, int ih, int ic, int groups, int pad, int stride,
                               int fs, int fn, int ow, int oh, int oc, int act,
                               int flags, int variant, int warmup, int iters, void *stream);

float ffgpu_irb_dev(const float *d_in, const float *d_w1, const float *d_wd, const float *d_w2,
                    const float *d_res, float *d_out, int batch, int iw, int ih, int ic, int ec, int oc,
                    int stride, int act1, int actd, int act2, int res_act, int warmup, int iters, void *stream);

float ffgpu_irb_flags_dev(const float *d_in, const float *d_w1, const float *d_wd, const float *d_w2,
                          const float *d_res, float *d_out, int batch, int iw, int ih, int ic, int ec, int oc,
                          int stride, int act1, int actd, int act2, int res_act, int flags, int warmup, int iters, void *stream);

int ffgpu_irb_thin_launch_text(int batch, int iw, int ih, int ic, int ec, int oc, int stride, int act1, int actd, int act2, int res_act,
                               int flags, char *buf, int cap);

int ffgpu_irb_plan_text(int batch, int iw, int ih, int ic, int ec, int oc, int stride, int act1, int actd, int act2, int res_act,
                        int flags, char *buf, int cap);

int ffgpu_irb_stage_plan_text(int batch, int iw, int ih, int blocks, int act1, int actd, int flags, char *buf, int cap);

int ffgpu_front_plan_text(int batch, int pw, int ph, int form, char *buf, int cap);

int ffgpu_irb_instantiations(char *buf, int cap);

int ffgpu_knobs_text(char *buf, int cap);

float ffgpu_dwpw_dev(const float *d_in, const float *d_wd, const float *d_wp, float *d_out, int batch, int iw, int ih,
                     int c, int oc, int fs, int actd, int actp, int warmup, int iters, void *stream);

size_t ffgpu_packed_records_bytes(int batch, int cap);
int    ffgpu_unpack_records(const void *block, int batch, int cap, ffgpu_frame_dets *out);
int    ffgpu_pack_records(const void *d_records, int nslots, long slot_stride_records, int batch, int cap, void *d_out, void *stream);

typedef struct {
    int image;
    int x0, y0;
    int reserved;
} ffgpu_tile;

#define FFGPU_MERGE_LDS_SLOTS 1024

size_t ffgpu_merge_tiles_scratch_bytes(int ntiles, int list_stride);
int    ffgpu_merge_tiles_dev(const void *d_records, const void *d_lists, int list_stride, const ffgpu_tile *tiles, int ntiles, int nimages,
                             float thresh, int use_min, void *d_out_records, void *d_out_lists, void *d_scratch, size_t scratch_bytes, void *stream);

int ffgpu_exec_merge_tiles(ffgpu_exec *ex, const ffgpu_tile *tiles, int ntiles, int nimages, void *stream);
int ffgpu_exec_merged_dev(ffgpu_exec *ex, void **dev_ptr, size_t *bytes);
int ffgpu_exec_read_merged(ffgpu_exec *ex, ffgpu_frame_dets *host_out, int max_images);
int ffgpu_exec_read_merged_boxes(ffgpu_exec *ex, int image, BBOX *host_out, int cap);

typedef struct { int x0, y0, w, h; } ffgpu_tile_rect;
int ffgpu_tile_plan(int img_w, int img_h, int tile_w, int tile_h, int overlap_x, int overlap_y, int align, ffgpu_tile_rect *out, int cap);

typedef struct {
    unsigned char color[4];
    const unsigned char *palette;
    int npalette;
    int thickness;
} ffgpu_draw_style;

int ffgpu_draw_boxes_bgr_dev (const void *d_records, const void *d_lists, int list_stride, const int *list_first,
                              const ffgpu_bgr_frame  *targets, int ntargets, const ffgpu_draw_style *style, void *stream);
int ffgpu_draw_boxes_nv12_dev(const void *d_records, const void *d_lists, int list_stride, const int *list_first,
                              const ffgpu_nv12_frame *targets, int ntargets, const ffgpu_draw_style *style, void *stream);

#define FFGPU_DRAW_ENTRIES 0
#define FFGPU_DRAW_MERGED  1
int ffgpu_exec_draw_bgr (ffgpu_exec *ex, int which, const ffgpu_bgr_frame  *targets, int ntargets, const ffgpu_draw_style *style, void *stream);
int ffgpu_exec_draw_nv12(ffgpu_exec *ex, int which, const ffgpu_nv12_frame *targets, int ntargets, const ffgpu_draw_style *style, void *stream);

#define FFGPU_CROP_F32 0
#define FFGPU_CROP_U8  1
typedef struct {
    int   out_w, out_h;
    int   form;
    int   per_target;
    float min_score;
    int   nclasses;
    const unsigned char *classes;
    int   margin_num, margin_den;
    float mean[3], norm[3];
    int   reserved;
} ffgpu_crop_spec;
typedef struct {
    int   target, box, type;
    float score;
    int   x0, y0, w, h;
    int   sw, sh, s1, s2;
} ffgpu_crop;

size_t ffgpu_crop_table_bytes(int capacity);
size_t ffgpu_crop_slot_bytes(int out_w, int out_h, int form);

int ffgpu_crop_boxes_bgr_dev (const void *d_records, const void *d_lists, int list_stride, const int *list_first, const ffgpu_bgr_frame  *sources,
                              int ntargets, const ffgpu_crop_spec *spec, void *d_out, void *d_table, int capacity, void *stream);
int ffgpu_crop_boxes_nv12_dev(const void *d_records, const void *d_lists, int list_stride, const int *list_first, const ffgpu_nv12_frame *sources,
                              int ntargets, const ffgpu_crop_spec *spec, void *d_out, void *d_table, int capacity, void *stream);

// ... 502 lines not shown
```

Measured before the change: 206,600.

## Compute narrow fused-block projection with packed FMAs and lane swaps instead of MFMA

Adds a packed-FMA variant of the wave-level fused inverted-residual kernel (k_irbw2_pk) for blocks with at most 8 output channels. The project stage uses v_pk_fma on two-wide vectors and cross-lane permlane swaps for the reduction, in place of fp32 16x16x4 MFMAs that waste most of their 16 output rows on such narrow outputs. It is selected at launch through a new knob that defaults on, and a text query reports which form a shape gets. The risks are extra VALU work and register pressure, plus a different summation order in the reduction.

```diff
diff --git a/ffcnn_amd/capi.py b/ffcnn_amd/capi.py
--- a/ffcnn_amd/capi.py
+++ b/ffcnn_amd/capi.py
@@ -302,7 +302,7 @@
            "ffgpu_exec_kernel_count", "ffgpu_exec_work_model", "ffgpu_exec_set_scale", "ffgpu_exec_forward_dev", "ffgpu_exec_forward_host",
            "ffgpu_exec_forward_bgr_dev", "ffgpu_exec_forward_bgr_frames_dev", "ffgpu_exec_forward_nv12_frames_dev", "ffgpu_exec_dets_dev", "ffgpu_exec_dets_host", "ffgpu_exec_set_ring", "ffgpu_exec_set_ring_strided", "ffgpu_exec_read_dets", "ffgpu_exec_read_layer", "ffgpu_exec_hash_layers",
            "ffgpu_exec_read_boxes", "ffgpu_exec_cand_capacity", "ffgpu_exec_graph_captures",
-           "ffgpu_exec_profile", "ffgpu_exec_profile_steps", "ffgpu_exec_step_model", "ffgpu_groupconv_dev", "ffgpu_groupconv_kernel_name", "ffgpu_groupconv_time_dev", "ffgpu_irb_dev", "ffgpu_irb_flags_dev", "ffgpu_irb_plan_text", "ffgpu_irb_thin_launch_text", "ffgpu_irb_stage_plan_text", "ffgpu_front_plan_text", "ffgpu_irb_instantiations", "ffgpu_knobs_text", "ffgpu_dwpw_dev", "ffgpu_packed_records_bytes", "ffgpu_pack_records", "ffgpu_unpack_records",
+           "ffgpu_exec_profile", "ffgpu_exec_profile_steps", "ffgpu_exec_step_model", "ffgpu_groupconv_dev", "ffgpu_groupconv_kernel_name", "ffgpu_groupconv_time_dev", "ffgpu_irb_dev", "ffgpu_irb_flags_dev", "ffgpu_irb_plan_text", "ffgpu_irb_thin_launch_text", "ffgpu_irbw_launch_text", "ffgpu_irb_stage_plan_text", "ffgpu_front_plan_text", "ffgpu_irb_instantiations", "ffgpu_knobs_text", "ffgpu_dwpw_dev", "ffgpu_packed_records_bytes", "ffgpu_pack_records", "ffgpu_unpack_records",
            "ffgpu_shard_range", "ffgpu_node_create", "ffgpu_node_destroy", "ffgpu_node_ndev", "ffgpu_node_shard", "ffgpu_node_set_scale",
            "ffgpu_node_input_dev", "ffgpu_node_input_slot_dev", "ffgpu_node_depth", "ffgpu_node_rccl_ranks", "ffgpu_node_forward", "ffgpu_node_forward_host",
            "ffgpu_node_submit", "ffgpu_node_wait", "ffgpu_node_run",
@@ -406,6 +406,7 @@
     L.ffgpu_irb_flags_dev.restype = C.c_float
     L.ffgpu_irb_flags_dev.argtypes = [vp] * 6 + [i] * 14 + [vp]
     L.ffgpu_irb_thin_launch_text.argtypes = [i] * 12 + [C.c_char_p, i]
+    L.ffgpu_irbw_launch_text.argtypes = [i] * 12 + [C.c_char_p, i]
     L.ffgpu_irb_plan_text.argtypes = [i] * 12 + [C.c_char_p, i]
     L.ffgpu_irb_stage_plan_text.argtypes = [i] * 7 + [C.c_char_p, i]
     L.ffgpu_front_plan_text.argtypes = [i] * 4 + [C.c_char_p, i]
@@ -1744,6 +1745,13 @@
     return buf.value.decode()
 
 
+def irbw_launch_text(shape, flags=0):
+    buf = C.create_string_buffer(256)
+    if lib().ffgpu_irbw_launch_text(*shape, flags, buf, len(buf)) < 0:
+        raise RuntimeError("ffgpu_irbw_launch_text failed: %s" % last_error())
+    return buf.value.decode()
+
+
 def irb_dev(d_in, d_w1, d_wd, d_w2, d_res, d_out, batch, iw, ih, ic, ec, oc, stride, act1=2, actd=2, act2=0, res_act=0,
             warmup=0, iters=0, stream=None, flags=0):
     us = lib().ffgpu_irb_flags_dev(d_in, d_w1, d_wd, d_w2, d_res, d_out, batch, iw, ih, ic, ec, oc, stride, act1, actd, act2, res_act, flags,
diff --git a/ffcnn_amd/csrc/ffgpu_conv_kernels.inc b/ffcnn_amd/csrc/ffgpu_conv_kernels.inc
--- a/ffcnn_amd/csrc/ffgpu_conv_kernels.inc
+++ b/ffcnn_amd/csrc/ffgpu_conv_kernels.inc
@@ -1081,13 +1081,13 @@
 }
 
 typedef int (*IrbwLaunch)(const IrbwP &, const IrbPlan &, hipStream_t);
-struct IrbwKernel { int KS1, OT, S, NSI, NSO; bool big, x3, xl; Knob gate; IrbwLaunch launch; };
+struct IrbwKernel { int KS1, OT, S, NSI, NSO; bool big, x3, xl; Knob gate; IrbwLaunch launch, proj; };
 #define IRBW_K(ks1, ot, st, nsi, gate) \
     { ks1, ot, st, nsi, 1, true, false, false, gate, irb_launch_t<IrbwP, k_irbw<ks1, ot, st, nsi, true>> }, \
     { ks1, ot, st, nsi, 1, false, false, false, gate, irb_launch_t<IrbwP, k_irbw<ks1, ot, st, nsi, false>> }
 static const IrbwKernel irbw_kernels[] = {
     { 2, 1, 1, 3, 2, true, true, false, K_NONE, irb_launch_t<IrbwP, k_irbw2<2, 3, true>> }, { 4, 1, 1, 3, 2, true, true, false, K_NONE, irb_launch_t<IrbwP, k_irbw2<4, 3, true>> },
-    { 2, 1, 1, 3, 2, true, false, false, K_NONE, irb_launch_t<IrbwP, k_irbw2<2, 3, false>> }, { 4, 1, 1, 3, 2, true, false, false, K_NONE, irb_launch_t<IrbwP, k_irbw2<4, 3, false>> },
+    { 2, 1, 1, 3, 2, true, false, false, K_NONE, irb_launch_t<IrbwP, k_irbw2<2, 3, false>>, irb_launch_t<IrbwP, k_irbw2_pk<2, 3>> }, { 4, 1, 1, 3, 2, true, false, false, K_NONE, irb_launch_t<IrbwP, k_irbw2<4, 3, false>> },
     { 12, 3, 1, 2, 1, true, true, true, K_NONE, irb_launch_t<IrbwP, k_irbw<12, 3, 1, 2, true, true, true>> },
     { 4, 2, 2, 4, 1, true, true, false, K_NONE, irb_launch_t<IrbwP, k_irbw<4, 2, 2, 4, true, true>> },
     { 6, 2, 1, 2, 1, true, true, false, K_NONE, irb_launch_t<IrbwP, k_irbw<6, 2, 1, 2, true, true>> },
@@ -1098,6 +1098,11 @@
 };
 #undef IRBW_K
 static const int irbw_nkernels = (int)(sizeof irbw_kernels / sizeof irbw_kernels[0]);
+
+static bool irbw_proj_form(const IrbDesc &d, const IrbPlan &c)
+{
+    return c.family == IRB_WAVE && d.oc <= 8 && irbw_kernels[c.inst].proj != nullptr && knob(K_IRBW_PROJ) != 0;
+}
 
 static bool irbw_has_kernel(int KS1, int OT, int S, int NSI)
 {
@@ -1595,7 +1600,17 @@
     if (knob(K_VERBOSE_IRB)) { char line[1024]; ffgpu_irb_plan_line(d, line, sizeof line); fprintf(stderr, "%s\n", line); }
     if (c.family == IRB_THIN) return launch_irb_thin(d, s);
     if (!d.pk) { ffgpu_set_error("irb: constants not packed"); return -1; }
-    return c.family == IRB_WAVE ? irbw_kernels[c.inst].launch(irbw_params(d), c, s) : irb_kernels[c.inst].launch(irb_params(d), c, s);
+    if (c.family == IRB_WAVE) return (irbw_proj_form(d, c) ? irbw_kernels[c.inst].proj : irbw_kernels[c.inst].launch)(irbw_params(d), c, s);
+    return irb_kernels[c.inst].launch(irb_params(d), c, s);
+}
+
+int ffgpu_irbw_launch_line(const IrbDesc &d, char *buf, size_t cap)
+{
+    const IrbPlan &c = d.plan;
+    if (c.family != IRB_WAVE) return snprintf(buf, cap, "unsupported");
+    char key[48];
+    irbw_key(irbw_kernels[c.inst], key, sizeof key);
+    return snprintf(buf, cap, "%s project=%s oc=%d grid=%d block=%d lds=%d", key, irbw_proj_form(d, c) ? "pk_fma" : "mfma", d.oc, c.grid, c.block, c.lds);
 }
 
 static bool irb_stage_params(const IrbDesc *blocks, int B, IrbStageP &p, size_t &lds)
diff --git a/ffcnn_amd/csrc/ffgpu_dev.hpp b/ffcnn_amd/csrc/ffgpu_dev.hpp
--- a/ffcnn_amd/csrc/ffgpu_dev.hpp
+++ b/ffcnn_amd/csrc/ffgpu_dev.hpp
@@ -74,6 +74,7 @@
 int    ffgpu_irb_pack(const IrbDesc &d, float *pk, hipStream_t s);
 int    ffgpu_launch_irb(const IrbDesc &d, hipStream_t s);
 int    ffgpu_irb_plan_line(const IrbDesc &d, char *buf, size_t cap);
+int    ffgpu_irbw_launch_line(const IrbDesc &d, char *buf, size_t cap);
 int    ffgpu_irb_thin_launch_line(const IrbDesc &d, char *buf, size_t cap);
 int    ffgpu_irb_keys(char *buf, size_t cap);
 #define IRBS_MAXB 8
diff --git a/ffcnn_amd/csrc/ffgpu_exec.hip b/ffcnn_amd/csrc/ffgpu_exec.hip
--- a/ffcnn_amd/csrc/ffgpu_exec.hip
+++ b/ffcnn_amd/csrc/ffgpu_exec.hip
@@ -1850,6 +1850,16 @@
     return ffgpu_irb_thin_launch_line(d, buf, (size_t)cap);
 }
 
+extern "C" int ffgpu_irbw_launch_text(int batch, int iw, int ih, int ic, int ec, int oc, int stride, int act1, int actd, int act2, int res_act, int flags, char *buf, int cap)
+{
+    if (!buf || cap < 1 || batch < 1 || iw < 1 || ih < 1 || stride < 1) { ffgpu_set_error("irbw_launch_text: bad arguments"); return -1; }
+    IrbDesc d{};
+    irb_fill(d, batch, iw, ih, ic, ec, oc, stride, act1, actd, act2, res_act);
+    d.flags = flags & FFGPU_CONCURRENT;
+    (void)ffgpu_irb_plan(d);
+    return ffgpu_irbw_launch_line(d, buf, (size_t)cap);
+}
+
 extern "C" float ffgpu_irb_dev(const float *d_in, const float *d_w1, const float *d_wd, const float *d_w2,
                                const float *d_res, float *d_out, int batch, int iw, int ih, int ic, int ec, int oc,
                                int stride, int act1, int actd, int act2, int res_act, int warmup, int iters, void *stream)
diff --git a/ffcnn_amd/csrc/ffgpu_irb_wave2.inc b/ffcnn_amd/csrc/ffgpu_irb_wave2.inc
--- a/ffcnn_amd/csrc/ffgpu_irb_wave2.inc
+++ b/ffcnn_amd/csrc/ffgpu_irb_wave2.inc
@@ -1,320 +1,27 @@
 #ifndef IRBW2_X3_KS2_MINB
 #define IRBW2_X3_KS2_MINB 2
 #endif
+__device__ __forceinline__ void irbw_swap32(float a, float b, float &lo, float &hi)
+{
+    const auto r = __builtin_amdgcn_permlane32_swap(__float_as_uint(a), __float_as_uint(b), false, false);
+    lo = __uint_as_float(r[0]); hi = __uint_as_float(r[1]);
+}
+__device__ __forceinline__ float irbw_swap16_add(float a, float b)
+{
+    const auto r = __builtin_amdgcn_permlane16_swap(__float_as_uint(a), __float_as_uint(b), false, false);
+    return __uint_as_float(r[0]) + __uint_as_float(r[1]);
+}
+
 template <int KS1, int NSI, bool X3>
 __global__ void __launch_bounds__(256, (X3 && KS1 == 2) ? IRBW2_X3_KS2_MINB : 2) k_irbw2(IrbwP p)
 {
-    constexpr int NM = X3 ? irbw_x3_nm(KS1) : 1;
-    extern __shared__ __attribute__((aligned(16))) float smem[];
-    const int tid = threadIdx.x, lane = tid & 63, wid = __builtin_amdgcn_readfirstlane(tid >> 6);
-    const int kq = lane >> 4, jq = lane & 15;
-    const float fl_act1 = act_floor(p.act1), fl_actd = act_floor(p.actd), fl_act2 = act_floor(p.act2), fl_res = act_floor(p.res_act);
-    constexpr int NPw = NSI * 64, NQ = NSI * 16, NSO = 2;
-    const int ecp = p.ngroups * 16;
-    const float *Wd = smem, *Sb1 = smem + ecp * 12, *Sb2 = Sb1 + ecp * 2;
-    float *Ew = smem + p.cs_floats + wid * (16 * NPw);
-    const v4f_w z = { 0.f, 0.f, 0.f, 0.f };
+    constexpr bool PK = KS1 < 0;
+#include "ffgpu_irb_wave2_body.inc"
+}
 
-    const int cs4 = p.cs_floats >> 2, nthr = (int)blockDim.x;
-    v4f_w cst[3];
-#pragma unroll
-    for (int u = 0; u < 3; u++) cst[u] = irbw_ld<v4f_w>(p.pk, (unsigned)(p.o_cs + 4 * min(tid + u * nthr, cs4 - 1)) * 4u);
-
-    const int tile = (p.xcd ? irbw_xcd_block((int)blockIdx.x, (int)gridDim.x) : (int)blockIdx.x) * p.WPB + wid;
-    const bool active = tile < (int)p.ntiles;
-    const int tt = active ? tile : 0;
-    const int trow = irbw_div(tt, p.m_tx), tx_i = tt - trow * p.tiles_x;
-    const int n = irbw_div(trow, p.m_ty), ty_i = trow - n * p.tiles_y;
-    const int oy0 = ty_i * p.TH, ox0 = tx_i * p.TWq * 4;
-    const int gy0 = oy0 - 1, gx0 = ox0 - 1;
-    const bool interior = gy0 >= 0 && gx0 >= 0 && gy0 + p.EH <= p.H && gx0 + p.EW <= p.W;
-
-    v4f_w xin[NSI][KS1];
-    unsigned mbits = 0;
-    {
-        const int plane = p.H * p.W;
-        bool anyfix = false;
-#pragma unroll
-        for (int si = 0; si < NSI; si++) {
-            const int e = si * 64 + 4 * jq;
-            const int iy = (int)__umulhi((unsigned)e, p.m_ew), ix = e - iy * p.EW;
-            const int gy = gy0 + iy, gx = gx0 + ix;
-            if (!interior) {
-                const bool rowok = (iy < p.EH) & ((unsigned)gy < (unsigned)p.H);
-#pragma unroll
-                for (int q = 0; q < 4; q++) mbits |= (rowok & ((unsigned)(gx + q) < (unsigned)p.W)) ? 1u << (si * 4 + q) : 0u;
-            }
-            const int rowidx = (n * p.H + min(max(gy, 0), p.H - 1)) * p.W + gx;
-#pragma unroll
-            for (int ks = 0; ks < KS1; ks++) {
-                const int idx = min(4 * ks + kq, p.ic - 1) * (p.N * plane) + rowidx;
-                const int cl = min(max(idx, 0), (int)p.in_elems - 4);
-                anyfix |= cl != idx;
-                xin[si][ks] = irbw_ld<v4f_w>(p.in, (unsigned)cl * 4u);
-            }
-        }
-        if (anyfix) {
-#pragma unroll
-            for (int si = 0; si < NSI; si++) {
-                const int e = si * 64 + 4 * jq;
-                const int iy = (int)__umulhi((unsigned)e, p.m_ew), ix = e - iy * p.EW;
-                const int rowidx = (n * p.H + min(max(gy0 + iy, 0), p.H - 1)) * p.W + gx0 + ix;
-#pragma unroll
-                for (int ks = 0; ks < KS1; ks++) {
-                    const int idx = min(4 * ks + kq, p.ic - 1) * (p.N * plane) + rowidx;
-                    const int d = min(max(idx, 0), (int)p.in_elems - 4) - idx;
-                    if (d != 0) {
-                        const v4f_w l = xin[si][ks];
-                        v4f_w w = z;
-#pragma unroll
-                        for (int q = 0; q < 4; q++) {
-                            const int s = q - d;
-                            w[q] = s == 0 ? l.x : (s == 1 ? l.y : (s == 2 ? l.z : (s == 3 ? l.w : 0.f)));
-                        }
-                        xin[si][ks] = w;
-                    }
-                }
-            }
-        }
-    }
-    if (4 * (KS1 - 1) + kq >= p.ic) {
-#pragma unroll
-        for (int si = 0; si < NSI; si++) xin[si][KS1 - 1] = z;
-    }
-    unsigned xp[X3 ? NSI : 1][4][3][X3 ? KS1 / 2 : 1];
-    if (X3) {
-        float amax = 0.f;
-#pragma unroll
-        for (int si = 0; si < NSI; si++)
-#pragma unroll
-            for (int ks = 0; ks < KS1; ks++) amax = x3_amax3(x3_amax3(amax, xin[si][ks][0], xin[si][ks][1]), xin[si][ks][2], xin[si][ks][3]);
-        auto split_tile = [&](auto INF) {
-#pragma unroll
-            for (int si = 0; si < NSI; si++)
-#pragma unroll
-                for (int q = 0; q < 4; q++) {
-                    unsigned b[3][KS1];
-#pragma unroll
-                    for (int ks = 0; ks < KS1; ks++) {
-                        const float x = xin[si][ks][q];
-                        const float r = x3_resid_t<decltype(INF)::value>(x);
-                        const float r2 = x3_resid2(r);
-                        b[0][ks] = __float_as_uint(x); b[1][ks] = __float_as_uint(r); b[2][ks] = __float_as_uint(r2);
-                    }
-#pragma unroll
-                    for (int pt = 0; pt < 3; pt++)
-#pragma unroll
-                        for (int pr = 0; pr < KS1 / 2; pr++) xp[si][q][pt][pr] = __builtin_amdgcn_perm(b[pt][2 * pr + 1], b[pt][2 * pr], 0x07060302u);
-                }
-        };
-        if (X3_INF_X_FUSED && x3_wave_has_inf(amax)) split_tile(std::true_type{}); else split_tile(std::false_type{});
-    }
-    auto bop = [&](int si, int q, int m) -> v8bf_w2 {
-        u4_w2 u;
-#pragma unroll
-        for (int d = 0; d < 4; d++) {
-            const IrbwX3Term t = irbw_x3_term(KS1, m, d);
-            u[d] = t.wp < 0 ? 0u : xp[X3 ? si : 0][q][t.xp][X3 ? t.pair : 0];
-        }
-        return __builtin_bit_cast(v8bf_w2, u);
-    };
-    int ebase[NSO], nvalid[NSO];
-    unsigned pbase[NSO];
-    const int typ = irbw_div(jq, p.m_twq), tq = jq - typ * p.TWq;
-#pragma unroll
-    for (int so = 0; so < NSO; so++) {
-        const int ty = 2 * typ + so;
-        const bool qvalid = ty < p.TH;
-        ebase[so] = qvalid ? ty * p.EW + tq * 4 : 0;
-        const int oy = oy0 + ty, ox = ox0 + tq * 4;
-        const bool valid = active && qvalid && oy < p.OH && ox < p.OW;
-        nvalid[so] = valid ? min(4, p.OW - ox) : 0;
-        pbase[so] = valid ? (unsigned)((n * p.OH + oy) * p.OW + ox) : 0u;
-    }
-    const unsigned ocs = (unsigned)(p.N * p.OH * p.OW);
-
-    struct W1T { float f[X3 ? 1 : KS1]; u4_w2 x[X3 ? NM : 1]; };
-    auto loadw = [&](int g, W1T &w1, float (&w2)[4]) {
-        if (X3) {
-#pragma unroll
-            for (int m = 0; m < NM; m++) w1.x[m] = irbw_ld<u4_w2>(p.pk, (unsigned)((g * NM + m) * 64 + lane) * 16u);
-        } else {
-#pragma unroll
-            for (int ks = 0; ks < KS1; ks++) w1.f[ks] = irbw_ld<float>(p.pk, (unsigned)((g * KS1 + ks) * 64 + lane) * 4u);
-        }
-#pragma unroll
-        for (int i = 0; i < 4; i++) w2[i] = irbw_ld<float>(p.pk, (unsigned)(p.o_w2 + (g * 4 + i) * 64 + lane) * 4u);
-    };
-    W1T w1a, w1b;
-    float w2a[4], w2b[4];
-    loadw(0, w1a, w2a);
-
-#pragma unroll
-    for (int u = 0; u < 3; u++) if (tid + u * nthr < cs4) reinterpret_cast<v4f_w *>(smem)[tid + u * nthr] = cst[u];
-    for (int i = tid + 3 * nthr; i < cs4; i += nthr)
-        reinterpret_cast<v4f_w *>(smem)[i] = irbw_ld<v4f_w>(p.pk, (unsigned)(p.o_cs + 4 * i) * 4u);
-    __syncthreads();
-
-    v4f_w acc[NSO][4];
-#pragma unroll
-    for (int so = 0; so < NSO; so++)
-#pragma unroll
-        for (int q = 0; q < 4; q++) acc[so][q] = z;
-    const unsigned mb = interior ? 0xffffffffu : mbits;
-
-    auto group = [&](int g, const W1T &w1, const float (&w2)[4]) {
-        const float *sbp = Sb1 + (g * 4 + kq) * 8;
-        const v4f_w S4 = *reinterpret_cast<const v4f_w *>(sbp), B4 = *reinterpret_cast<const v4f_w *>(sbp + 4);
-        const v2f_w sc[2] = { { S4.x, S4.y }, { S4.z, S4.w } }, bi[2] = { { B4.x, B4.y }, { B4.z, B4.w } };
-#pragma unroll
-        for (int si = 0; si < NSI; si++) {
-            v4f_w a4[4] = { z, z, z, z };
-            if (X3) {
-#pragma unroll
-                for (int m = 0; m < NM; m++) {
-                    const v8bf_w2 A = __builtin_bit_cast(v8bf_w2, w1.x[m]);
-#pragma unroll
-                    for (int q = 0; q < 4; q++) a4[q] = __builtin_amdgcn_mfma_f32_16x16x32_bf16(A, bop(si, q, m), a4[q], 0, 0, 0);
-                }
-            } else {
-#pragma unroll
-                for (int ks = 0; ks < KS1; ks++) {
-                    a4[0] = __builtin_amdgcn_mfma_f32_16x16x4f32(w1.f[ks], xin[si][ks].x, a4[0], 0, 0, 0);
-                    a4[1] = __builtin_amdgcn_mfma_f32_16x16x4f32(w1.f[ks], xin[si][ks].y, a4[1], 0, 0, 0);
-                    a4[2] = __builtin_amdgcn_mfma_f32_16x16x4f32(w1.f[ks], xin[si][ks].z, a4[2], 0, 0, 0);
-                    a4[3] = __builtin_amdgcn_mfma_f32_16x16x4f32(w1.f[ks], xin[si][ks].w, a4[3], 0, 0, 0);
-                }
-            }
-#pragma unroll
-            for (int rp = 0; rp < 2; rp++) {
-                v2f_w y[4];
-#pragma unroll
-                for (int q = 0; q < 4; q++) {
-                    const v2f_w a = rp == 0 ? (v2f_w){ a4[q].x, a4[q].y } : (v2f_w){ a4[q].z, a4[q].w };
-                    const v2f_w t = a * sc[rp] + bi[rp];
-                    const v2f_w u = t * p.act1;
-                    const bool in = (mb >> (si * 4 + q)) & 1u;
-                    y[q] = (v2f_w){ in ? act_max(t.x, u.x, fl_act1) : 0.f, in ? act_max(t.y, u.y, fl_act1) : 0.f };
-                }
-                float *dst = Ew + ((2 * kq + rp) * 2 * NQ + si * 16 + jq) * 4;
-                *reinterpret_cast<v4f_w *>(dst) = (v4f_w){ y[0].x, y[0].y, y[1].x, y[1].y };
-                *reinterpret_cast<v4f_w *>(dst + NQ * 4) = (v4f_w){ y[2].x, y[2].y, y[3].x, y[3].y };
-            }
-        }
-#pragma unroll
-        for (int m = 0; m < 2; m++) {
-            const int pr = 2 * kq + m;
-            const float *wdp = Wd + (g * 8 + pr) * 24;
-            v4f_w T[6];
-#pragma unroll
-            for (int i = 0; i < 6; i++) T[i] = *reinterpret_cast<const v4f_w *>(wdp + 4 * i);
-            const v2f_w tap[9] = { { T[0].x, T[0].y }, { T[0].z, T[0].w }, { T[1].x, T[1].y }, { T[1].z, T[1].w }, { T[2].x, T[2].y },
-                                   { T[2].z, T[2].w }, { T[3].x, T[3].y }, { T[3].z, T[3].w }, { T[4].x, T[4].y } };
-            const v2f_w sd = { T[4].z, T[4].w }, bd = { T[5].x, T[5].y };
-            const float *ep = Ew + (pr * 2 * NQ + (ebase[0] >> 2)) * 4;
-            v2f_w dv[NSO][4];
-#pragma unroll
-            for (int so = 0; so < NSO; so++)
-#pragma unroll
-                for (int q = 0; q < 4; q++) dv[so][q] = (v2f_w){ 0.f, 0.f };
-#pragma unroll
-            for (int r = 0; r < 4; r++) {
-                const float *row = ep + r * p.EW;
-                v2f_w x[6];
-#pragma unroll
-                for (int i = 0; i < 3; i++) {
-                    const v4f_w u = *reinterpret_cast<const v4f_w *>(row + ((i & 1) * NQ + (i >> 1)) * 4);
-                    x[2 * i] = (v2f_w){ u.x, u.y }; x[2 * i + 1] = (v2f_w){ u.z, u.w };
-                }
-                if (r < 3) {
-#pragma unroll
-                    for (int q = 0; q < 4; q++)
-#pragma unroll
-                        for (int kx = 0; kx < 3; kx++) dv[0][q] += tap[r * 3 + kx] * x[q + kx];
-                }
-                if (r >= 1) {
-#pragma unroll
-                    for (int q = 0; q < 4; q++)
-#pragma unroll
-                        for (int kx = 0; kx < 3; kx++) dv[1][q] += tap[(r - 1) * 3 + kx] * x[q + kx];
-                }
-            }
-#pragma unroll
-            for (int so = 0; so < NSO; so++) {
-                v2f_w bq[4];
-#pragma unroll
-                for (int q = 0; q < 4; q++) {
-                    const v2f_w t = dv[so][q] * sd + bd;
-                    const v2f_w u = t * p.actd;
-                    bq[q] = (v2f_w){ act_max(t.x, u.x, fl_actd), act_max(t.y, u.y, fl_actd) };
-                }
-#pragma unroll
-                for (int j = 0; j < 2; j++) {
-                    const float a = w2[2 * m + j];
-                    acc[so][0] = __builtin_amdgcn_mfma_f32_16x16x4f32(a, j ? bq[0].y : bq[0].x, acc[so][0], 0, 0, 0);
-                    acc[so][1] = __builtin_amdgcn_mfma_f32_16x16x4f32(a, j ? bq[1].y : bq[1].x, acc[so][1], 0, 0, 0);
-                    acc[so][2] = __builtin_amdgcn_mfma_f32_16x16x4f32(a, j ? bq[2].y : bq[2].x, acc[so][2], 0, 0, 0);
-                    acc[so][3] = __builtin_amdgcn_mfma_f32_16x16x4f32(a, j ? bq[3].y : bq[3].x, acc[so][3], 0, 0, 0);
-                }
-            }
-        }
-    };
-
-    if (active) {
-        for (int g = 0; g < p.ngroups; g += 2) {
-            loadw(min(g + 1, p.ngroups - 1), w1b, w2b);
-            __builtin_amdgcn_sched_barrier(0);
-            group(g, w1a, w2a);
-            if (g + 1 < p.ngroups) {
-                loadw(min(g + 2, p.ngroups - 1), w1a, w2a);
-                __builtin_amdgcn_sched_barrier(0);
-                group(g + 1, w1b, w2b);
-            }
-        }
-    }
-
-    const bool lin_out = p.act2 == 1.f && p.res_act == 1.f;
-    auto rows_out = [&](auto MODE) {
-        constexpr int M = decltype(MODE)::value;
-#pragma unroll
-        for (int so = 0; so < NSO; so++) {
-            v4f_w res[4];
-            if (M == 0 || (M == 2 && p.residual)) {
-#pragma unroll
-                for (int r = 0; r < 4; r++) {
-                    const unsigned off = ((unsigned)min(4 * kq + r, p.oc - 1) * ocs + pbase[so]) * 4u;
-                    if (p.vec == 4) res[r] = irbw_ld<v4f_w>(p.residual, nvalid[so] == 4 ? off : 0u);
-                    else {
-#pragma unroll
-                        for (int q = 0; q < 4; q++) res[r][q] = irbw_ld<float>(p.residual, q < nvalid[so] ? off + 4u * q : 0u);
-                    }
-                }
-            }
-#pragma unroll
-            for (int r = 0; r < 4; r++) {
-                const int o = 4 * kq + r, oo = min(o, p.oc - 1);
-                const v2f_w sb = *reinterpret_cast<const v2f_w *>(Sb2 + 2 * oo);
-                v4f_w v = pw_fma4_apart(acc[so][0][r], acc[so][1][r], acc[so][2][r], acc[so][3][r], sb.x, sb.y);
-                if (M == 0) v += res[r];
-                if (M == 2) {
-#pragma unroll
-                    for (int q = 0; q < 4; q++) {
-                        v[q] = irbw_act(v[q], p.act2, fl_act2);
-                        if (p.residual) v[q] = irbw_act(v[q] + res[r][q], p.res_act, fl_res);
-                    }
-                }
-                const unsigned off = ((unsigned)oo * ocs + pbase[so]) * 4u;
-                if (o < p.oc) {
-                    if (p.vec == 4) { if (nvalid[so] == 4) irbw_st<v4f_w>(p.out, off, v); }
-                    else {
-#pragma unroll
-                        for (int q = 0; q < 4; q++) if (q < nvalid[so]) irbw_st<float>(p.out, off + 4u * q, v[q]);
-                    }
-                }
-            }
-        }
-    };
-    if (lin_out && p.residual) rows_out(std::integral_constant<int, 0>());
-    else if (lin_out) rows_out(std::integral_constant<int, 1>());
-    else rows_out(std::integral_constant<int, 2>());
+template <int KS1, int NSI>
+__global__ void __launch_bounds__(256, 2) k_irbw2_pk(IrbwP p)
+{
+    constexpr bool X3 = KS1 < 0, PK = KS1 > 0;
+#include "ffgpu_irb_wave2_body.inc"
 }
diff --git a/ffcnn_amd/csrc/ffgpu_irb_wave2_body.inc b/ffcnn_amd/csrc/ffgpu_irb_wave2_body.inc
--- /dev/null
+++ b/ffcnn_amd/csrc/ffgpu_irb_wave2_body.inc
@@ -0,0 +1,378 @@
+    constexpr int NM = X3 ? irbw_x3_nm(KS1) : 1;
+    extern __shared__ __attribute__((aligned(16))) float smem[];
+    const int tid = threadIdx.x, lane = tid & 63, wid = __builtin_amdgcn_readfirstlane(tid >> 6);
+    const int kq = lane >> 4, jq = lane & 15;
+    const float fl_act1 = act_floor(p.act1), fl_actd = act_floor(p.actd), fl_act2 = act_floor(p.act2), fl_res = act_floor(p.res_act);
+    constexpr int NPw = NSI * 64, NQ = NSI * 16, NSO = 2;
+    const int ecp = p.ngroups * 16;
+    const float *Wd = smem, *Sb1 = smem + ecp * 12, *Sb2 = Sb1 + ecp * 2;
+    float *Ew = smem + p.cs_floats + wid * (16 * NPw);
+    const v4f_w z = { 0.f, 0.f, 0.f, 0.f };
+
+    const int cs4 = p.cs_floats >> 2, nthr = (int)blockDim.x;
+    v4f_w cst[3];
+#pragma unroll
+    for (int u = 0; u < 3; u++) cst[u] = irbw_ld<v4f_w>(p.pk, (unsigned)(p.o_cs + 4 * min(tid + u * nthr, cs4 - 1)) * 4u);
+
+    const int tile = (p.xcd ? irbw_xcd_block((int)blockIdx.x, (int)gridDim.x) : (int)blockIdx.x) * p.WPB + wid;
+    const bool active = tile < (int)p.ntiles;
+    const int tt = active ? tile : 0;
+    const int trow = irbw_div(tt, p.m_tx), tx_i = tt - trow * p.tiles_x;
+    const int n = irbw_div(trow, p.m_ty), ty_i = trow - n * p.tiles_y;
+    const int oy0 = ty_i * p.TH, ox0 = tx_i * p.TWq * 4;
+    const int gy0 = oy0 - 1, gx0 = ox0 - 1;
+    const bool interior = gy0 >= 0 && gx0 >= 0 && gy0 + p.EH <= p.H && gx0 + p.EW <= p.W;
+
+    v4f_w xin[NSI][KS1];
+    unsigned mbits = 0;
+    {
+        const int plane = p.H * p.W;
+        bool anyfix = false;
+#pragma unroll
+        for (int si = 0; si < NSI; si++) {
+            const int e = si * 64 + 4 * jq;
+            const int iy = (int)__umulhi((unsigned)e, p.m_ew), ix = e - iy * p.EW;
+            const int gy = gy0 + iy, gx = gx0 + ix;
+            if (!interior) {
+                const bool rowok = (iy < p.EH) & ((unsigned)gy < (unsigned)p.H);
+#pragma unroll
+                for (int q = 0; q < 4; q++) mbits |= (rowok & ((unsigned)(gx + q) < (unsigned)p.W)) ? 1u << (si * 4 + q) : 0u;
+            }
+            const int rowidx = (n * p.H + min(max(gy, 0), p.H - 1)) * p.W + gx;
+#pragma unroll
+            for (int ks = 0; ks < KS1; ks++) {
+                const int idx = min(4 * ks + kq, p.ic - 1) * (p.N * plane) + rowidx;
+                const int cl = min(max(idx, 0), (int)p.in_elems - 4);
+                anyfix |= cl != idx;
+                xin[si][ks] = irbw_ld<v4f_w>(p.in, (unsigned)cl * 4u);
+            }
+        }
+        if (anyfix) {
+#pragma unroll
+            for (int si = 0; si < NSI; si++) {
+                const int e = si * 64 + 4 * jq;
+                const int iy = (int)__umulhi((unsigned)e, p.m_ew), ix = e - iy * p.EW;
+                const int rowidx = (n * p.H + min(max(gy0 + iy, 0), p.H - 1)) * p.W + gx0 + ix;
+#pragma unroll
+                for (int ks = 0; ks < KS1; ks++) {
+                    const int idx = min(4 * ks + kq, p.ic - 1) * (p.N * plane) + rowidx;
+                    const int d = min(max(idx, 0), (int)p.in_elems - 4) - idx;
+                    if (d != 0) {
+                        const v4f_w l = xin[si][ks];
+                        v4f_w w = z;
+#pragma unroll
+                        for (int q = 0; q < 4; q++) {
+                            const int s = q - d;
+                            w[q] = s == 0 ? l.x : (s == 1 ? l.y : (s == 2 ? l.z : (s == 3 ? l.w : 0.f)));
+                        }
+                        xin[si][ks] = w;
+                    }
+                }
+            }
+        }
+    }
+    if (4 * (KS1 - 1) + kq >= p.ic) {
+#pragma unroll
+        for (int si = 0; si < NSI; si++) xin[si][KS1 - 1] = z;
+    }
+    unsigned xp[X3 ? NSI : 1][4][3][X3 ? KS1 / 2 : 1];
+    if (X3) {
+        float amax = 0.f;
+#pragma unroll
+        for (int si = 0; si < NSI; si++)
+#pragma unroll
+            for (int ks = 0; ks < KS1; ks++) amax = x3_amax3(x3_amax3(amax, xin[si][ks][0], xin[si][ks][1]), xin[si][ks][2], xin[si][ks][3]);
+        auto split_tile = [&](auto INF) {
+#pragma unroll
+            for (int si = 0; si < NSI; si++)
+#pragma unroll
+                for (int q = 0; q < 4; q++) {
+                    unsigned b[3][KS1];
+#pragma unroll
+                    for (int ks = 0; ks < KS1; ks++) {
+                        const float x = xin[si][ks][q];
+                        const float r = x3_resid_t<decltype(INF)::value>(x);
+                        const float r2 = x3_resid2(r);
+                        b[0][ks] = __float_as_uint(x); b[1][ks] = __float_as_uint(r); b[2][ks] = __float_as_uint(r2);
+                    }
+#pragma unroll
+                    for (int pt = 0; pt < 3; pt++)
+#pragma unroll
+                        for (int pr = 0; pr < KS1 / 2; pr++) xp[si][q][pt][pr] = __builtin_amdgcn_perm(b[pt][2 * pr + 1], b[pt][2 * pr], 0x07060302u);
+                }
+        };
+        if (X3_INF_X_FUSED && x3_wave_has_inf(amax)) split_tile(std::true_type{}); else split_tile(std::false_type{});
+    }
+    auto bop = [&](int si, int q, int m) -> v8bf_w2 {
+        u4_w2 u;
+#pragma unroll
+        for (int d = 0; d < 4; d++) {
+            const IrbwX3Term t = irbw_x3_term(KS1, m, d);
+            u[d] = t.wp < 0 ? 0u : xp[X3 ? si : 0][q][t.xp][X3 ? t.pair : 0];
+        }
+        return __builtin_bit_cast(v8bf_w2, u);
+    };
+    int ebase[NSO], nvalid[NSO];
+    unsigned pbase[NSO];
+    const int typ = irbw_div(jq, p.m_twq), tq = jq - typ * p.TWq;
+#pragma unroll
+    for (int so = 0; so < NSO; so++) {
+        const int ty = 2 * typ + so;
+        const bool qvalid = ty < p.TH;
+        ebase[so] = qvalid ? ty * p.EW + tq * 4 : 0;
+        const int oy = oy0 + ty, ox = ox0 + tq * 4;
+        const bool valid = active && qvalid && oy < p.OH && ox < p.OW;
+        nvalid[so] = valid ? min(4, p.OW - ox) : 0;
+        pbase[so] = valid ? (unsigned)((n * p.OH + oy) * p.OW + ox) : 0u;
+    }
+    const unsigned ocs = (unsigned)(p.N * p.OH * p.OW);
+
+    struct W1T { float f[X3 ? 1 : KS1]; u4_w2 x[X3 ? NM : 1]; };
+    auto loadw = [&](int g, W1T &w1, float (&w2)[4]) {
+        if (X3) {
+#pragma unroll
+            for (int m = 0; m < NM; m++) w1.x[m] = irbw_ld<u4_w2>(p.pk, (unsigned)((g * NM + m) * 64 + lane) * 16u);
+        } else {
+#pragma unroll
+            for (int ks = 0; ks < KS1; ks++) w1.f[ks] = irbw_ld<float>(p.pk, (unsigned)((g * KS1 + ks) * 64 + lane) * 4u);
+        }
+        if constexpr (!PK) {
+#pragma unroll
+            for (int i = 0; i < 4; i++) w2[i] = irbw_ld<float>(p.pk, (unsigned)(p.o_w2 + (g * 4 + i) * 64 + lane) * 4u);
+        }
+    };
+    const int kp = kq & 1, hq = kq >> 1;
+    auto loadp = [&](int g, int i, v4f_w (&wp)[2][2]) {
+#pragma unroll
+        for (int s = 0; s < 2; s++)
+#pragma unroll
+            for (int h = 0; h < 2; h++) wp[s][h] = irbw_ld<v4f_w>(p.pk, (unsigned)(p.o_w2 + (g * 4 + i) * 64 + 16 * (kp + 2 * s) + 4 * h) * 4u);
+    };
+    W1T w1a, w1b;
+    float w2a[4], w2b[4];
+    loadw(0, w1a, w2a);
+
+#pragma unroll
+    for (int u = 0; u < 3; u++) if (tid + u * nthr < cs4) reinterpret_cast<v4f_w *>(smem)[tid + u * nthr] = cst[u];
+    for (int i = tid + 3 * nthr; i < cs4; i += nthr)
+        reinterpret_cast<v4f_w *>(smem)[i] = irbw_ld<v4f_w>(p.pk, (unsigned)(p.o_cs + 4 * i) * 4u);
+    __syncthreads();
+
+    v4f_w acc[NSO][4];
+#pragma unroll
+    for (int so = 0; so < NSO; so++)
+#pragma unroll
+        for (int q = 0; q < 4; q++) acc[so][q] = z;
+    v2f_w pacc[4][4];
+    if constexpr (PK) {
+#pragma unroll
+        for (int q = 0; q < 4; q++)
+#pragma unroll
+            for (int pp = 0; pp < 4; pp++) pacc[q][pp] = (v2f_w){ 0.f, 0.f };
+    }
+    const int npair = (p.oc + 1) >> 1;
+    const unsigned mb = interior ? 0xffffffffu : mbits;
+
+    auto group = [&](int g, const W1T &w1, const float (&w2)[4]) {
+        const float *sbp = Sb1 + (g * 4 + kq) * 8;
+        const v4f_w S4 = *reinterpret_cast<const v4f_w *>(sbp), B4 = *reinterpret_cast<const v4f_w *>(sbp + 4);
+        const v2f_w sc[2] = { { S4.x, S4.y }, { S4.z, S4.w } }, bi[2] = { { B4.x, B4.y }, { B4.z, B4.w } };
+        v4f_w wp0[2][2], wp1[2][2];
+        if constexpr (PK) loadp(g, 0, wp0);
+#pragma unroll
+        for (int si = 0; si < NSI; si++) {
+            v4f_w a4[4] = { z, z, z, z };
+            if (X3) {
+#pragma unroll
+                for (int m = 0; m < NM; m++) {
+                    const v8bf_w2 A = __builtin_bit_cast(v8bf_w2, w1.x[m]);
+#pragma unroll
+                    for (int q = 0; q < 4; q++) a4[q] = __builtin_amdgcn_mfma_f32_16x16x32_bf16(A, bop(si, q, m), a4[q], 0, 0, 0);
+                }
+            } else {
+#pragma unroll
+                for (int ks = 0; ks < KS1; ks++) {
+                    a4[0] = __builtin_amdgcn_mfma_f32_16x16x4f32(w1.f[ks], xin[si][ks].x, a4[0], 0, 0, 0);
+                    a4[1] = __builtin_amdgcn_mfma_f32_16x16x4f32(w1.f[ks], xin[si][ks].y, a4[1], 0, 0, 0);
+                    a4[2] = __builtin_amdgcn_mfma_f32_16x16x4f32(w1.f[ks], xin[si][ks].z, a4[2], 0, 0, 0);
+                    a4[3] = __builtin_amdgcn_mfma_f32_16x16x4f32(w1.f[ks], xin[si][ks].w, a4[3], 0, 0, 0);
+                }
+            }
+#pragma unroll
+            for (int rp = 0; rp < 2; rp++) {
+                v2f_w y[4];
+#pragma unroll
+                for (int q = 0; q < 4; q++) {
+                    const v2f_w a = rp == 0 ? (v2f_w){ a4[q].x, a4[q].y } : (v2f_w){ a4[q].z, a4[q].w };
+                    const v2f_w t = a * sc[rp] + bi[rp];
+                    const v2f_w u = t * p.act1;
+                    const bool in = (mb >> (si * 4 + q)) & 1u;
+                    y[q] = (v2f_w){ in ? act_max(t.x, u.x, fl_act1) : 0.f, in ? act_max(t.y, u.y, fl_act1) : 0.f };
+                }
+                float *dst = Ew + ((2 * kq + rp) * 2 * NQ + si * 16 + jq) * 4;
+                *reinterpret_cast<v4f_w *>(dst) = (v4f_w){ y[0].x, y[0].y, y[1].x, y[1].y };
+                *reinterpret_cast<v4f_w *>(dst + NQ * 4) = (v4f_w){ y[2].x, y[2].y, y[3].x, y[3].y };
+            }
+        }
+#pragma unroll
+        for (int m = 0; m < 2; m++) {
+            const int pr = 2 * kq + m;
+            const float *wdp = Wd + (g * 8 + pr) * 24;
+            v4f_w T[6];
+#pragma unroll
+            for (int i = 0; i < 6; i++) T[i] = *reinterpret_cast<const v4f_w *>(wdp + 4 * i);
+            const v2f_w tap[9] = { { T[0].x, T[0].y }, { T[0].z, T[0].w }, { T[1].x, T[1].y }, { T[1].z, T[1].w }, { T[2].x, T[2].y },
+                                   { T[2].z, T[2].w }, { T[3].x, T[3].y }, { T[3].z, T[3].w }, { T[4].x, T[4].y } };
+            const v2f_w sd = { T[4].z, T[4].w }, bd = { T[5].x, T[5].y };
+            const float *ep = Ew + (pr * 2 * NQ + (ebase[0] >> 2)) * 4;
+            v2f_w dv[NSO][4];
+#pragma unroll
+            for (int so = 0; so < NSO; so++)
+#pragma unroll
+                for (int q = 0; q < 4; q++) dv[so][q] = (v2f_w){ 0.f, 0.f };
+#pragma unroll
+            for (int r = 0; r < 4; r++) {
+                const float *row = ep + r * p.EW;
+                v2f_w x[6];
+#pragma unroll
+                for (int i = 0; i < 3; i++) {
+                    const v4f_w u = *reinterpret_cast<const v4f_w *>(row + ((i & 1) * NQ + (i >> 1)) * 4);
+                    x[2 * i] = (v2f_w){ u.x, u.y }; x[2 * i + 1] = (v2f_w){ u.z, u.w };
+                }
+                if (r < 3) {
+#pragma unroll
+                    for (int q = 0; q < 4; q++)
+#pragma unroll
+                        for (int kx = 0; kx < 3; kx++) dv[0][q] += tap[r * 3 + kx] * x[q + kx];
+                }
+                if (r >= 1) {
+#pragma unroll
+                    for (int q = 0; q < 4; q++)
+#pragma unroll
+                        for (int kx = 0; kx < 3; kx++) dv[1][q] += tap[(r - 1) * 3 + kx] * x[q + kx];
+                }
+            }
+            if constexpr (PK) {
+                v2f_w bq[NSO][4];
+#pragma unroll
+                for (int so = 0; so < NSO; so++)
+#pragma unroll
+                    for (int q = 0; q < 4; q++) {
+                        const v2f_w t = dv[so][q] * sd + bd;
+                        const v2f_w u = t * p.actd;
+                        bq[so][q] = (v2f_w){ act_max(t.x, u.x, fl_actd), act_max(t.y, u.y, fl_actd) };
+                    }
+                loadp(g, 2 * m + 1, wp1);
+                float ra[2][4], rb[2][4];
+#pragma unroll
+                for (int j = 0; j < 2; j++)
+#pragma unroll
+                    for (int q = 0; q < 4; q++) irbw_swap32(bq[0][q][j], bq[1][q][j], ra[j][q], rb[j][q]);
+#pragma unroll
+                for (int j = 0; j < 2; j++) {
+                    const v4f_w (&wp)[2][2] = j ? wp1 : wp0;
+#pragma unroll
+                    for (int s = 0; s < 2; s++)
+#pragma unroll
+                        for (int pp = 0; pp < 4; pp++) {
+                            if (pp >= npair) break;
+                            const v4f_w w4 = wp[s][pp >> 1];
+                            const v2f_w w = (pp & 1) ? (v2f_w){ w4.z, w4.w } : (v2f_w){ w4.x, w4.y };
+#pragma unroll
+                            for (int q = 0; q < 4; q++) pacc[q][pp] += w * (s ? rb[j][q] : ra[j][q]);
+                        }
+                }
+                if (m == 0) loadp(g, 2, wp0);
+            } else {
+#pragma unroll
+            for (int so = 0; so < NSO; so++) {
+                v2f_w bq[4];
+#pragma unroll
+                for (int q = 0; q < 4; q++) {
+                    const v2f_w t = dv[so][q] * sd + bd;
+                    const v2f_w u = t * p.actd;
+                    bq[q] = (v2f_w){ act_max(t.x, u.x, fl_actd), act_max(t.y, u.y, fl_actd) };
+                }
+#pragma unroll
+                for (int j = 0; j < 2; j++) {
+                    const float a = w2[2 * m + j];
+                    acc[so][0] = __builtin_amdgcn_mfma_f32_16x16x4f32(a, j ? bq[0].y : bq[0].x, acc[so][0], 0, 0, 0);
+                    acc[so][1] = __builtin_amdgcn_mfma_f32_16x16x4f32(a, j ? bq[1].y : bq[1].x, acc[so][1], 0, 0, 0);
+                    acc[so][2] = __builtin_amdgcn_mfma_f32_16x16x4f32(a, j ? bq[2].y : bq[2].x, acc[so][2], 0, 0, 0);
+                    acc[so][3] = __builtin_amdgcn_mfma_f32_16x16x4f32(a, j ? bq[3].y : bq[3].x, acc[so][3], 0, 0, 0);
+                }
+            }
+            }
+        }
+    };
+
+    if (active) {
+        for (int g = 0; g < p.ngroups; g += 2) {
+            loadw(min(g + 1, p.ngroups - 1), w1b, w2b);
+            __builtin_amdgcn_sched_barrier(0);
+            group(g, w1a, w2a);
+            if (g + 1 < p.ngroups) {
+                loadw(min(g + 2, p.ngroups - 1), w1a, w2a);
+                __builtin_amdgcn_sched_barrier(0);
+                group(g + 1, w1b, w2b);
+            }
+        }
+    }
+
+    float red[4][4];
+    if constexpr (PK) {
+#pragma unroll
+        for (int q = 0; q < 4; q++)
+#pragma unroll
+            for (int r = 0; r < 4; r++) red[q][r] = irbw_swap16_add(pacc[q][r >> 1][r & 1], pacc[q][2 + (r >> 1)][r & 1]);
+    }
+    constexpr int NSR = PK ? 1 : NSO;
+    const int kqo = PK ? kp : kq;
+    auto accv = [&](int so, int q, int r) -> float { if constexpr (PK) return red[q][r]; else return acc[so][q][r]; };
+    auto pb = [&](int so) -> unsigned { if constexpr (PK) return hq ? pbase[1] : pbase[0]; else return pbase[so]; };
+    auto nv = [&](int so) -> int { if constexpr (PK) return hq ? nvalid[1] : nvalid[0]; else return nvalid[so]; };
+
+    const bool lin_out = p.act2 == 1.f && p.res_act == 1.f;
+    auto rows_out = [&](auto MODE) {
+        constexpr int M = decltype(MODE)::value;
+#pragma unroll
+        for (int so = 0; so < NSR; so++) {
+            v4f_w res[4];
+            if (M == 0 || (M == 2 && p.residual)) {
+#pragma unroll
+                for (int r = 0; r < 4; r++) {
+                    const unsigned off = ((unsigned)min(4 * kqo + r, p.oc - 1) * ocs + pb(so)) * 4u;
+                    if (p.vec == 4) res[r] = irbw_ld<v4f_w>(p.residual, nv(so) == 4 ? off : 0u);
+                    else {
+#pragma unroll
+                        for (int q = 0; q < 4; q++) res[r][q] = irbw_ld<float>(p.residual, q < nv(so) ? off + 4u * q : 0u);
+                    }
+                }
+            }
+#pragma unroll
+            for (int r = 0; r < 4; r++) {
+                const int o = 4 * kqo + r, oo = min(o, p.oc - 1);
+                const v2f_w sb = *reinterpret_cast<const v2f_w *>(Sb2 + 2 * oo);
+                v4f_w v = pw_fma4_apart(accv(so, 0, r), accv(so, 1, r), accv(so, 2, r), accv(so, 3, r), sb.x, sb.y);
+                if (M == 0) v += res[r];
+                if (M == 2) {
+#pragma unroll
+                    for (int q = 0; q < 4; q++) {
+                        v[q] = irbw_act(v[q], p.act2, fl_act2);
+                        if (p.residual) v[q] = irbw_act(v[q] + res[r][q], p.res_act, fl_res);
+                    }
+                }
+                const unsigned off = ((unsigned)oo * ocs + pb(so)) * 4u;
+                if (o < p.oc) {
+                    if (p.vec == 4) { if (nv(so) == 4) irbw_st<v4f_w>(p.out, off, v); }
+                    else {
+#pragma unroll
+                        for (int q = 0; q < 4; q++) if (q < nv(so)) irbw_st<float>(p.out, off + 4u * q, v[q]);
+                    }
+                }
+            }
+        }
+    };
+    if (lin_out && p.residual) rows_out(std::integral_constant<int, 0>());
+    else if (lin_out) rows_out(std::integral_constant<int, 1>());
+    else rows_out(std::integral_constant<int, 2>());
diff --git a/ffcnn_amd/csrc/ffgpu_knobs.hpp b/ffcnn_amd/csrc/ffgpu_knobs.hpp
--- a/ffcnn_amd/csrc/ffgpu_knobs.hpp
+++ b/ffcnn_amd/csrc/ffgpu_knobs.hpp
@@ -100,6 +100,7 @@
     X(IRBW2_TWQ,         "FFGPU_IRBW2_TWQ",         INT,  0,             TUNING,  "k_irbw2: tile width in quads (with FFGPU_IRBW2_TH; 0: searched)") \
     X(IRBW2_TH,          "FFGPU_IRBW2_TH",          INT,  0,             TUNING,  "k_irbw2: tile height (with FFGPU_IRBW2_TWQ; 0: searched)") \
     X(IRBW2_MIN_TILES,   "FFGPU_IRBW2_MIN_TILES",   INT,  768,           TUNING,  "k_irbw2: fewest tiles the planner takes it for") \
+    X(IRBW_PROJ,         "FFGPU_IRBW_PROJ",         INT,  1,             TUNING,  "fused blocks of at most 8 output channels: 0 keeps the project stage on fp32 MFMAs instead of packed FMAs (the instantiations that have the form); read at launch") \
     X(IRBW_WPB,          "FFGPU_IRBW_WPB",          INT,  0,             TUNING,  "k_irbw: tiles per workgroup without a group split, 1 .. 8 (0: 4 or 8 by LDS)") \
     X(IRBW_HALF,         "FFGPU_IRBW_HALF",         INT,  1,             PRODUCT, "0: a last group of at most 8 real expanded channels is computed as a whole group") \
     X(IRBW_XCD,          "FFGPU_IRBW_XCD",          INT,  3,             PRODUCT, "fused blocks walk their tiles XCD by XCD; bit 0: one-wave-per-tile launches, bit 1: group-split launches") \
diff --git a/include/ffcnn_hip.h b/include/ffcnn_hip.h
--- a/include/ffcnn_hip.h
+++ b/include/ffcnn_hip.h
@@ -163,6 +163,9 @@
 int ffgpu_irb_thin_launch_text(int batch, int iw, int ih, int ic, int ec, int oc, int stride, int act1, int actd, int act2, int res_act,
                                int flags, char *buf, int cap);
 
+int ffgpu_irbw_launch_text(int batch, int iw, int ih, int ic, int ec, int oc, int stride, int act1, int actd, int act2, int res_act,
+                           int flags, char *buf, int cap);
+
 int ffgpu_irb_plan_text(int batch, int iw, int ih, int ic, int ec, int oc, int stride, int act1, int actd, int act2, int res_act,
                         int flags, char *buf, int cap);
 
```

New measurement: 206,700, median of 4. About the same (+0.1%).
